# chzchzchz/raftsql

Measured on AMD Instinct MI355X. Metric: quorum decisions/sec (commit+vote) across G groups, higher is better.
Workload: dtype u64

## Files before the change

go/raftq/engine_more.go:

```go
package raftq

import "C"

import "unsafe"

func ABIVersion() int { return int(C.raftq_abi_version()) }

func Quorum(peers uint32) uint32 { return uint32(C.raftq_quorum(C.uint32_t(peers))) }

func (e *Engine) NGroups() uint64 { return uint64(C.raftq_groups(e.h)) }
func (e *Engine) NPeers() uint32  { return uint32(C.raftq_peers(e.h)) }

func (e *Engine) SelfMax() (int, error) {
	var slot C.int32_t
	if err := e.err(C.raftq_self_max(e.h, &slot)); err != nil {
		return -1, err
	}
	return int(slot), nil
}

func (e *Engine) Narrow() (bool, error) {
	var valid C.int32_t
	if err := e.err(C.raftq_narrow(e.h, &valid)); err != nil {
		return false, err
	}
	return valid != 0, nil
}

func (e *Engine) NarrowRebuild() error { return e.err(C.raftq_narrow_rebuild(e.h)) }

func (e *Engine) SetStream(stream unsafe.Pointer) error { return e.err(C.raftq_set_stream(e.h, stream)) }
func (e *Engine) Stream() unsafe.Pointer                { return C.raftq_get_stream(e.h) }

type TermDelta struct{ Group, CurTerm, FirstIdxCurTerm uint64 }

func (e *Engine) ApplyTermDeltas(d []TermDelta) error {
	if len(d) == 0 {
		return nil
	}
	return e.err(C.raftq_apply_term_deltas(e.h, (*C.raftq_term_delta_t)(unsafe.Pointer(&d[0])), C.uint64_t(len(d))))
}

func (e *Engine) CommitAdvance(gated bool, committedOut []uint64) (changed uint64, err error) {
	var p *C.uint64_t
	if committedOut != nil {
		p = (*C.uint64_t)(unsafe.Pointer(&committedOut[0]))
	}
	g := C.int(0)
	if gated {
		g = 1
	}
	var n C.uint64_t
	err = e.err(C.raftq_commit_advance(e.h, g, p, &n))
	return uint64(n), err
}

func (e *Engine) VoteTally(outcomeOut []uint8) (Counts, error) {
	var p *C.uint8_t
	if outcomeOut != nil {
		p = (*C.uint8_t)(unsafe.Pointer(&outcomeOut[0]))
	}
	var c C.raftq_counts_t
	if err := e.err(C.raftq_vote_tally(e.h, p, &c)); err != nil {
		return Counts{}, err
	}
	return Counts{uint64(c.n_changed), uint64(c.n_won), uint64(c.n_lost)}, nil
}

func (e *Engine) ReadVotes(out []uint8) error {
	return e.err(C.raftq_read_votes(e.h, (*C.uint8_t)(unsafe.Pointer(&out[0]))))
}

func (e *Engine) SetTimers(electionTick, heartbeatTick uint32, seed uint64) error {
	return e.err(C.raftq_set_timers(e.h, C.uint32_t(electionTick), C.uint32_t(heartbeatTick), C.uint64_t(seed)))
}

type TickCounts struct{ Hup, Beat uint64 }

func (e *Engine) Tick(wantCounts bool) (TickCounts, error) {
	var c C.raftq_tick_counts_t
	if !wantCounts {
		return TickCounts{}, e.err(C.raftq_tick(e.h, nil))
	}
	err := e.err(C.raftq_tick(e.h, &c))
	return TickCounts{uint64(c.n_hup), uint64(c.n_beat)}, err
}

func (e *Engine) CollectHups(out []uint64) (uint64, error) {
	var n C.uint64_t
	var p *C.uint64_t
	if len(out) > 0 {
		p = (*C.uint64_t)(unsafe.Pointer(&out[0]))
	}
	rc := C.raftq_collect_hups(e.h, p, C.uint64_t(len(out)), &n)
	return uint64(n), e.err(rc)
}

func (e *Engine) TickCollect(hups, beats []uint64) (nHup, nBeat uint64, err error) {
	var hp, bp *C.uint64_t
	if len(hups) > 0 {
		hp = (*C.uint64_t)(unsafe.Pointer(&hups[0]))
	}
	if len(beats) > 0 {
		bp = (*C.uint64_t)(unsafe.Pointer(&beats[0]))
	}
	var nh, nb C.uint64_t
	err = e.err(C.raftq_tick_collect(e.h, hp, C.uint64_t(len(hups)), &nh, bp, C.uint64_t(len(beats)), &nb))
	return uint64(nh), uint64(nb), err
}

const TickBeatBitmap = uint(C.RAFTQ_TICK_BEAT_BITMAP)

// ... 218 lines not shown
```

include/raftq.h:

```cpp
#ifndef RAFTQ_H
#define RAFTQ_H

#include <stddef.h>
#include <stdint.h>

#ifdef __cplusplus
extern "C" {
#endif

#define RAFTQ_ABI_VERSION 1
#define RAFTQ_MAX_PEERS 9

#define RAFTQ_OK 0
#define RAFTQ_EINVAL (-1)
#define RAFTQ_ENOMEM (-2)
#define RAFTQ_EHIP (-3)
#define RAFTQ_ESTATE (-4)
#define RAFTQ_ENODEV (-5)

#define RAFTQ_SWEEP_COMMIT 0x01u
#define RAFTQ_SWEEP_GATED 0x02u
#define RAFTQ_SWEEP_VOTES 0x04u
#define RAFTQ_SWEEP_NO_ADOPT 0x08u
#define RAFTQ_SWEEP_LDS 0x10u
// ... 16 lines not shown
  uint64_t match;
  uint32_t peer;
  uint32_t _pad;
} raftq_delta_t;

typedef struct raftq_vote_delta {
  uint64_t group;
  uint32_t peer;
  uint8_t vote;
  uint8_t _pad[3];
} raftq_vote_delta_t;

typedef struct raftq_term_delta {
  uint64_t group;
  uint64_t cur_term;
  uint64_t first_idx_cur_term;
} raftq_term_delta_t;

typedef struct raftq_advance {
  uint64_t group;
  uint64_t old_commit;
  uint64_t new_commit;
} raftq_advance_t;

typedef struct raftq_delta16 {
  uint64_t match;
  uint32_t group;
  uint32_t peer;
} raftq_delta16_t;
typedef struct raftq_advance16 {
  uint64_t new_commit;
  uint32_t group;
  uint32_t advanced_by;
} raftq_advance16_t;

int raftq_abi_version(void);
int raftq_device_count(int* n);
uint32_t raftq_quorum(uint32_t n_peers);

#define RAFTQ_MAX_GROUPS (1ull << 30)
int raftq_create(int device, uint64_t n_groups, uint32_t n_peers, raftq_t** out);
void raftq_destroy(raftq_t* h);
uint64_t raftq_groups(const raftq_t* h);
uint32_t raftq_peers(const raftq_t* h);
const char* raftq_last_error(const raftq_t* h);

int raftq_set_stream(raftq_t* h, void* stream);
void* raftq_get_stream(const raftq_t* h);

int raftq_load_match(raftq_t* h, const uint64_t* match ,
                     const uint64_t* committed );
int raftq_load_terms(raftq_t* h, const uint64_t* cur_term ,
                     const uint64_t* first_idx_cur_term );
int raftq_load_votes(raftq_t* h, const uint8_t* votes );

int raftq_apply_deltas(raftq_t* h, const raftq_delta_t* d, uint64_t n);
int raftq_apply_vote_deltas(raftq_t* h, const raftq_vote_delta_t* d, uint64_t n);
int raftq_apply_term_deltas(raftq_t* h, const raftq_term_delta_t* d, uint64_t n);

typedef struct raftq_voter_delta {
  uint64_t group;
  uint16_t voters;
  uint16_t reset;
  uint32_t _pad;
} raftq_voter_delta_t;
int raftq_load_voters(raftq_t* h, const uint16_t* voters);
int raftq_apply_voter_deltas(raftq_t* h, const raftq_voter_delta_t* d, uint64_t n);
int raftq_read_voters(raftq_t* h, uint16_t* voters_out);

int raftq_step_async(raftq_t* h, unsigned flags);
int raftq_wait(raftq_t* h, raftq_counts_t* counts);

int raftq_commit_advance(raftq_t* h, int gated, uint64_t* committed_out ,
                         uint64_t* n_changed );
int raftq_vote_tally(raftq_t* h, uint8_t* outcome_out ,
                     raftq_counts_t* counts );

int raftq_read_committed(raftq_t* h, uint64_t* committed_out );
int raftq_read_outcome(raftq_t* h, uint8_t* outcome_out );
int raftq_read_match(raftq_t* h, uint64_t* match_out );
int raftq_self_max(raftq_t* h, int32_t* slot_out);
int raftq_narrow(raftq_t* h, int32_t* valid_out);
int raftq_narrow_rebuild(raftq_t* h);
int raftq_read_votes(raftq_t* h, uint8_t* votes_out );
int raftq_collect_changed(raftq_t* h, raftq_advance_t* out, uint64_t cap, uint64_t* n);

#define RAFTQ_ROLE_FOLLOWER 0
#define RAFTQ_ROLE_CANDIDATE 1
#define RAFTQ_ROLE_LEADER 2
#define RAFTQ_ROLE_PRE_CANDIDATE 3
typedef struct raftq_tick_counts {
  uint64_t n_hup;
  uint64_t n_beat;
} raftq_tick_counts_t;
int raftq_set_timers(raftq_t* h, uint32_t election_tick, uint32_t heartbeat_tick, uint64_t seed);
int raftq_load_roles(raftq_t* h, const uint8_t* role , const uint32_t* elapsed );
int raftq_tick_set_voters(raftq_t* h, int on);
int raftq_tick(raftq_t* h, raftq_tick_counts_t* counts);
int raftq_read_tick(raftq_t* h, uint8_t* action , uint32_t* elapsed , uint8_t* role );
int raftq_collect_hups(raftq_t* h, uint64_t* groups, uint64_t cap, uint64_t* n);
int raftq_collect_beats(raftq_t* h, uint64_t* groups, uint64_t cap, uint64_t* n);
int raftq_tick_collect(raftq_t* h, uint64_t* hups, uint64_t hup_cap, uint64_t* n_hup, uint64_t* beats, uint64_t beat_cap,
                       uint64_t* n_beat);

#define RAFTQ_TICK_BEAT_BITMAP 1u
int raftq_tick_collect_lists(raftq_t* h, unsigned flags, uint64_t hup_cap, uint64_t beat_cap, uint64_t* n_hup, uint64_t* n_beat);
int raftq_last_tick_lists(raftq_t* h, const uint32_t** hups, uint64_t* n_hups, const uint32_t** beats, uint64_t* n_beats,
                          const uint64_t** beat_bitmap, uint64_t* bitmap_words);
int raftq_set_check_quorum(raftq_t* h, int on);
int raftq_tick_set_checks(raftq_t* h, uint64_t chk_cap);
int raftq_last_tick_checks(raftq_t* h, const uint32_t** checks, uint64_t* n_listed, uint64_t* n_total);
int raftq_load_activity(raftq_t* h, const uint16_t* active , const uint32_t* lead_elapsed );
int raftq_read_activity(raftq_t* h, uint16_t* active , uint32_t* lead_elapsed );
int raftq_collect_checks(raftq_t* h, uint64_t* groups, uint64_t cap, uint64_t* n);

int raftq_set_pre_vote(raftq_t* h, int on);

int raftq_set_lead_transfer(raftq_t* h, int on);
int raftq_load_transfer(raftq_t* h, const uint8_t* transferee );
int raftq_read_transfer(raftq_t* h, uint8_t* transferee );

#define RAFTQ_READ_SAFE 1
#define RAFTQ_READ_LEASE 2
int raftq_set_read_index(raftq_t* h, int mode);
int raftq_load_reads(raftq_t* h, const uint32_t* seq , const uint32_t* acked );
int raftq_read_reads(raftq_t* h, uint32_t* seq, uint32_t* acked, uint32_t* confirmed );

int raftq_campaign(raftq_t* h, const uint64_t* groups, uint64_t n, uint32_t self_peer);

int raftq_cycle(raftq_t* h, const raftq_delta_t* deltas, uint64_t n_deltas,
                const raftq_vote_delta_t* vote_deltas, uint64_t n_vote_deltas, unsigned flags,
                raftq_advance_t* advances_out, uint64_t cap, uint64_t* n_advanced,
                raftq_counts_t* counts);

int raftq_stage(raftq_t* h, uint64_t n_deltas, uint64_t n_vote_deltas, raftq_delta_t** deltas,
                raftq_vote_delta_t** vote_deltas);
int raftq_last_advances(raftq_t* h, const raftq_advance_t** list, uint64_t* n_listed);

int raftq_cycle_packed(raftq_t* h, const raftq_delta16_t* deltas, uint64_t n_deltas,
                       const raftq_vote_delta_t* vote_deltas, uint64_t n_vote_deltas, unsigned flags,
                       raftq_advance16_t* advances_out, uint64_t cap, uint64_t* n_advanced,
                       raftq_counts_t* counts);
int raftq_stage_packed(raftq_t* h, uint64_t n_deltas, uint64_t n_vote_deltas, raftq_delta16_t** deltas,
                       raftq_vote_delta_t** vote_deltas);
int raftq_last_advances_packed(raftq_t* h, const raftq_advance16_t** list, uint64_t* n_listed);

#define RAFTQ_CYCLE_SEGMENTED 0x200u
int raftq_last_advance_segments(raftq_t* h, const raftq_advance16_t** recs, const uint32_t** counts, uint32_t* n_segments,
                                uint64_t* stride);

typedef struct raftq_set raftq_set_t;
#define RAFTQ_SET_GRID 0
#define RAFTQ_SET_PERSISTENT 1
int raftq_set_create(raftq_t* const* handles, uint32_t n, raftq_set_t** out);
int raftq_set_create_voters(raftq_t* const* handles, uint32_t n, raftq_set_t** out);
void raftq_set_destroy(raftq_set_t* s);
uint32_t raftq_set_size(const raftq_set_t* s);
const char* raftq_set_last_error(const raftq_set_t* s);
void* raftq_set_get_stream(const raftq_set_t* s);
int raftq_set_mode(raftq_set_t* s, int mode, uint32_t persist_workgroups);
int raftq_set_sweep_async(raftq_set_t* s, unsigned flags);
int raftq_set_tick(raftq_set_t* s);
int raftq_set_wait(raftq_set_t* s, raftq_counts_t* per_member, raftq_counts_t* total);
int raftq_set_timer_begin(raftq_set_t* s);
int raftq_set_timer_end(raftq_set_t* s, float* elapsed_ms);
int raftq_sweep_many_async(raftq_t* const* handles, uint32_t n, unsigned flags);
// ... 13 lines not shown
```

raftsql_amd/_lib.py:

```python
from __future__ import annotations

import ctypes as C
import os

_HERE = os.path.dirname(os.path.abspath(__file__))
LIB_PATH = os.environ.get("RAFTQ_LIB") or os.path.join(_HERE, "libraftq.so")

RAFTQ_OK = 0
RAFTQ_EINVAL, RAFTQ_ENOMEM, RAFTQ_EHIP, RAFTQ_ESTATE, RAFTQ_ENODEV = -1, -2, -3, -4, -5

SWEEP_COMMIT = 0x01
SWEEP_GATED = 0x02
SWEEP_VOTES = 0x04
SWEEP_NO_ADOPT = 0x08
SWEEP_LDS = 0x10
SWEEP_CHANGED = 0x20
SWEEP_STREAM = 0x40
SWEEP_CACHED = 0x80
CYCLE_TRUSTED = 0x100
TICK_BEAT_BITMAP = 1
CYCLE_SEGMENTED = 0x200
SET_GRID, SET_PERSISTENT = 0, 1

MAX_PEERS = 9
READ_SAFE, READ_LEASE = 1, 2


class Counts(C.Structure):
    _fields_ = [("n_changed", C.c_uint64), ("n_won", C.c_uint64), ("n_lost", C.c_uint64)]


class TickCounts(C.Structure):
    _fields_ = [("n_hup", C.c_uint64), ("n_beat", C.c_uint64)]


class Delta(C.Structure):
    _fields_ = [("group", C.c_uint64), ("match", C.c_uint64), ("peer", C.c_uint32), ("_pad", C.c_uint32)]


class VoteDelta(C.Structure):
    _fields_ = [("group", C.c_uint64), ("peer", C.c_uint32), ("vote", C.c_uint8), ("_pad", C.c_uint8 * 3)]


class VoterDelta(C.Structure):
    _fields_ = [("group", C.c_uint64), ("voters", C.c_uint16), ("reset", C.c_uint16), ("_pad", C.c_uint32)]


class Advance(C.Structure):
    _fields_ = [("group", C.c_uint64), ("old_commit", C.c_uint64), ("new_commit", C.c_uint64)]


_H = C.c_void_p
_SIGS = [
    ("raftq_abi_version", C.c_int, []),
    ("raftq_device_count", C.c_int, [C.POINTER(C.c_int)]),
    ("raftq_quorum", C.c_uint32, [C.c_uint32]),
    ("raftq_create", C.c_int, [C.c_int, C.c_uint64, C.c_uint32, C.POINTER(_H)]),
    ("raftq_destroy", None, [_H]),
    ("raftq_groups", C.c_uint64, [_H]),
    ("raftq_peers", C.c_uint32, [_H]),
    ("raftq_last_error", C.c_char_p, [_H]),
    ("raftq_set_stream", C.c_int, [_H, C.c_void_p]),
    ("raftq_get_stream", C.c_void_p, [_H]),
    ("raftq_load_match", C.c_int, [_H, C.c_void_p, C.c_void_p]),
    ("raftq_load_terms", C.c_int, [_H, C.c_void_p, C.c_void_p]),
    ("raftq_load_votes", C.c_int, [_H, C.c_void_p]),
    ("raftq_apply_deltas", C.c_int, [_H, C.c_void_p, C.c_uint64]),
    ("raftq_apply_vote_deltas", C.c_int, [_H, C.c_void_p, C.c_uint64]),
    ("raftq_apply_term_deltas", C.c_int, [_H, C.c_void_p, C.c_uint64]),
    ("raftq_load_voters", C.c_int, [_H, C.c_void_p]),
    ("raftq_apply_voter_deltas", C.c_int, [_H, C.c_void_p, C.c_uint64]),
    ("raftq_read_voters", C.c_int, [_H, C.c_void_p]),
    ("raftq_step_async", C.c_int, [_H, C.c_uint]),
    ("raftq_wait", C.c_int, [_H, C.POINTER(Counts)]),
    ("raftq_commit_advance", C.c_int, [_H, C.c_int, C.c_void_p, C.POINTER(C.c_uint64)]),
    ("raftq_vote_tally", C.c_int, [_H, C.c_void_p, C.POINTER(Counts)]),
    ("raftq_read_committed", C.c_int, [_H, C.c_void_p]),
    ("raftq_read_outcome", C.c_int, [_H, C.c_void_p]),
    ("raftq_read_match", C.c_int, [_H, C.c_void_p]),
    ("raftq_self_max", C.c_int, [_H, C.POINTER(C.c_int32)]),
    ("raftq_narrow", C.c_int, [_H, C.POINTER(C.c_int32)]),
    ("raftq_narrow_rebuild", C.c_int, [_H]),
    ("raftq_read_votes", C.c_int, [_H, C.c_void_p]),
    ("raftq_collect_changed", C.c_int, [_H, C.c_void_p, C.c_uint64, C.POINTER(C.c_uint64)]),
    ("raftq_set_timers", C.c_int, [_H, C.c_uint32, C.c_uint32, C.c_uint64]),
    ("raftq_load_roles", C.c_int, [_H, C.c_void_p, C.c_void_p]),
    ("raftq_tick_set_voters", C.c_int, [_H, C.c_int]),
    ("raftq_tick_set_checks", C.c_int, [_H, C.c_uint64]),
    ("raftq_last_tick_checks", C.c_int, [_H, C.POINTER(C.c_void_p), C.POINTER(C.c_uint64), C.POINTER(C.c_uint64)]),
    ("raftq_tick", C.c_int, [_H, C.POINTER(TickCounts)]),
    ("raftq_read_tick", C.c_int, [_H, C.c_void_p, C.c_void_p, C.c_void_p]),
    ("raftq_collect_hups", C.c_int, [_H, C.c_void_p, C.c_uint64, C.POINTER(C.c_uint64)]),
    ("raftq_collect_beats", C.c_int, [_H, C.c_void_p, C.c_uint64, C.POINTER(C.c_uint64)]),
    ("raftq_tick_collect", C.c_int, [_H, C.c_void_p, C.c_uint64, C.POINTER(C.c_uint64), C.c_void_p, C.c_uint64, C.POINTER(C.c_uint64)]),
    ("raftq_tick_collect_lists", C.c_int, [_H, C.c_uint, C.c_uint64, C.c_uint64, C.POINTER(C.c_uint64), C.POINTER(C.c_uint64)]),
    ("raftq_last_tick_lists", C.c_int, [_H, C.POINTER(C.c_void_p), C.POINTER(C.c_uint64), C.POINTER(C.c_void_p), C.POINTER(C.c_uint64),
                                        C.POINTER(C.c_void_p), C.POINTER(C.c_uint64)]),
    ("raftq_set_check_quorum", C.c_int, [_H, C.c_int]),
    ("raftq_set_pre_vote", C.c_int, [_H, C.c_int]),
    ("raftq_set_lead_transfer", C.c_int, [_H, C.c_int]),
    ("raftq_load_transfer", C.c_int, [_H, C.c_void_p]),
    ("raftq_read_transfer", C.c_int, [_H, C.c_void_p]),
    ("raftq_set_read_index", C.c_int, [_H, C.c_int]),
    ("raftq_load_reads", C.c_int, [_H, C.c_void_p, C.c_void_p]),
    ("raftq_read_reads", C.c_int, [_H, C.c_void_p, C.c_void_p, C.c_void_p]),
    ("raftq_load_activity", C.c_int, [_H, C.c_void_p, C.c_void_p]),
    ("raftq_read_activity", C.c_int, [_H, C.c_void_p, C.c_void_p]),
    ("raftq_collect_checks", C.c_int, [_H, C.c_void_p, C.c_uint64, C.POINTER(C.c_uint64)]),
    ("raftq_campaign", C.c_int, [_H, C.c_void_p, C.c_uint64, C.c_uint32]),
    ("raftq_cycle", C.c_int, [_H, C.c_void_p, C.c_uint64, C.c_void_p, C.c_uint64, C.c_uint, C.c_void_p, C.c_uint64,
                              C.POINTER(C.c_uint64), C.POINTER(Counts)]),
    ("raftq_stage", C.c_int, [_H, C.c_uint64, C.c_uint64, C.POINTER(C.c_void_p), C.POINTER(C.c_void_p)]),
    ("raftq_last_advances", C.c_int, [_H, C.POINTER(C.c_void_p), C.POINTER(C.c_uint64)]),
    ("raftq_cycle_packed", C.c_int, [_H, C.c_void_p, C.c_uint64, C.c_void_p, C.c_uint64, C.c_uint, C.c_void_p, C.c_uint64,
                                     C.POINTER(C.c_uint64), C.POINTER(Counts)]),
    ("raftq_stage_packed", C.c_int, [_H, C.c_uint64, C.c_uint64, C.POINTER(C.c_void_p), C.POINTER(C.c_void_p)]),
    ("raftq_last_advances_packed", C.c_int, [_H, C.POINTER(C.c_void_p), C.POINTER(C.c_uint64)]),
    ("raftq_last_advance_segments", C.c_int, [_H, C.POINTER(C.c_void_p), C.POINTER(C.c_void_p), C.POINTER(C.c_uint32), C.POINTER(C.c_uint64)]),
    ("raftq_set_create", C.c_int, [C.POINTER(_H), C.c_uint32, C.POINTER(_H)]),
    ("raftq_set_create_voters", C.c_int, [C.POINTER(_H), C.c_uint32, C.POINTER(_H)]),
    ("raftq_set_destroy", None, [_H]),
    ("raftq_set_size", C.c_uint32, [_H]),
    ("raftq_set_last_error", C.c_char_p, [_H]),
    ("raftq_set_get_stream", C.c_void_p, [_H]),
    ("raftq_set_mode", C.c_int, [_H, C.c_int, C.c_uint32]),
    ("raftq_set_sweep_async", C.c_int, [_H, C.c_uint]),
    ("raftq_set_wait", C.c_int, [_H, C.c_void_p, C.POINTER(Counts)]),
    ("raftq_set_tick", C.c_int, [_H]),
    ("raftq_set_timer_begin", C.c_int, [_H]),
    ("raftq_set_timer_end", C.c_int, [_H, C.POINTER(C.c_float)]),
    ("raftq_sweep_many_async", C.c_int, [C.POINTER(_H), C.c_uint32, C.c_uint]),
    ("raftq_clone_state", C.c_int, [_H, _H]),
    ("raftq_timer_begin", C.c_int, [_H]),
    ("raftq_timer_end", C.c_int, [_H, C.POINTER(C.c_float)]),
    ("raftq_host_alloc", C.c_int, [C.POINTER(C.c_void_p), C.c_uint64]),
    ("raftq_host_free", None, [C.c_void_p]),
]
EXPORTS = [s[0] for s in _SIGS]


class StepCounts(C.Structure):
    _fields_ = [("n_msgs", C.c_uint64), ("n_groups_touched", C.c_uint64)]


_STEP_SIGS = [
    ("raftq_set_self", C.c_int, [_H, C.c_uint32]),
    ("raftq_load_node", C.c_int, [_H, C.c_void_p, C.c_void_p, C.c_void_p, C.c_void_p, C.c_void_p]),
    ("raftq_read_node", C.c_int, [_H, C.c_void_p, C.c_void_p, C.c_void_p, C.c_void_p, C.c_void_p, C.c_void_p]),
    ("raftq_step_batch", C.c_int, [_H, C.c_void_p, C.c_uint64, C.c_void_p, C.POINTER(StepCounts)]),
    ("raftq_apply_log_deltas", C.c_int, [_H, C.c_void_p, C.c_uint64, C.c_void_p]),
    ("raftq_apply_log_deltas_nowait", C.c_int, [_H, C.c_void_p, C.c_uint64]),
    ("raftq_step_submit", C.c_int, [_H, C.c_void_p, C.c_uint64]),
    ("raftq_step_collect", C.c_int, [_H, C.c_void_p, C.POINTER(StepCounts)]),
    ("raftq_step_stage", C.c_int, [_H, C.c_uint64, C.POINTER(C.c_void_p)]),
    ("raftq_step_stage_packed", C.c_int, [_H, C.c_uint64, C.POINTER(C.c_void_p)]),
    ("raftq_step_submit_packed", C.c_int, [_H, C.c_void_p, C.c_uint64]),
    ("raftq_step_results", C.c_int, [_H, C.POINTER(C.c_void_p), C.POINTER(C.c_uint64)]),
    ("raftq_step_set_compact", C.c_int, [_H, C.c_int]),
    ("raftq_step_set_msg_flags", C.c_int, [_H, C.c_int]),
    ("raftq_step_set_voters", C.c_int, [_H, C.c_int]),
    ("raftq_step_set_props", C.c_int, [_H, C.c_int]),
    ("raftq_step_results_c", C.c_int, [_H, C.POINTER(C.c_void_p), C.POINTER(C.c_uint64)]),
    ("raftq_step_results_s", C.c_int, [_H, C.POINTER(C.c_void_p), C.POINTER(C.c_uint64)]),
]
STEP_EXPORTS = [s[0] for s in _STEP_SIGS]
# ... 86 lines not shown
```

raftsql_amd/csrc/raftq_capi.hip:

```cpp
#include "raftq.h"

#include <hip/hip_runtime.h>

#include <algorithm>
#include <atomic>
#include <mutex>
#include <chrono>
#include <cstdlib>
#include <cstdio>
#include <cstring>
#include <new>
#include <string>
#include <type_traits>
#include <unordered_set>
#include <vector>

#include "raftq_internal.hpp"

#ifndef RAFTQ_GPL
#define RAFTQ_GPL 4
#endif
#ifndef RAFTQ_AUTO_STREAM_BYTES
#define RAFTQ_AUTO_STREAM_BYTES (128ull << 20)
#endif
// ... 56 lines not shown
    case 6: return f(Const<6>{});
    case 7: return f(Const<7>{});
    case 8: return f(Const<8>{});
    case 9: return f(Const<9>{});
    default: return hipErrorInvalidValue;
  }
}

template <class F>
hipError_t with_flag_form(unsigned flags, F f) {
  const bool commit = flags & (RAFTQ_SWEEP_COMMIT | RAFTQ_SWEEP_GATED);
  const bool gated = flags & RAFTQ_SWEEP_GATED;
  const bool votes = flags & RAFTQ_SWEEP_VOTES;
  if (commit && gated) return votes ? f(FlagForm<true, true, true>{}) : f(FlagForm<true, true, false>{});
  if (commit) return votes ? f(FlagForm<true, false, true>{}) : f(FlagForm<true, false, false>{});
  return f(FlagForm<false, false, true>{});
}

template <class F>
hipError_t with_policy(int nt, F f) {
  if (nt == 3) return f(Const<kLdNT | kStNT>{});
  if (nt == 1) return f(Const<kLdNT>{});
  return f(Const<0>{});
}

constexpr int set_gpl(int n_peers) { return n_peers <= 5 ? 8 : 2; }

template <int N, class Form, int POLICY>
hipError_t launch_reg(const SweepLaunch& L, hipStream_t s) {
  constexpr bool COMMIT = Form::commit, GATED = Form::gated, VOTES = Form::votes;
  const unsigned tiles = (unsigned)(L.gpad / kTile);
  if (L.tab == nullptr) {
    hipLaunchKernelGGL((sweep_kernel<N, kGPL, COMMIT, GATED, VOTES, POLICY, true>), dim3(tiles), dim3(kBlock), 0, s, *L.one);
  } else if (L.persist_wgs == 0) {
    constexpr int G = set_gpl(N);
    hipLaunchKernelGGL((sweep_set_kernel<N, G, COMMIT, GATED, VOTES, POLICY, true>),
                       dim3((unsigned)(L.gpad / ((uint64_t)kBlock * G)), L.members), dim3(kBlock), 0, s, L.tab, L.want_bits);
  } else {
    const uint32_t total = tiles * L.members;
    hipLaunchKernelGGL((sweep_persist_kernel<N, kGPL, COMMIT, GATED, VOTES, POLICY, true>),
                       dim3(std::min<uint32_t>(L.persist_wgs, total)), dim3(kBlock), 0, s, L.tab, tiles, total, L.want_bits);
  }
  return hipGetLastError();
}

template <int N, class Form>
hipError_t launch_lds(const SweepArgs& a, uint64_t gpad, hipStream_t s) {
  if constexpr (Form::commit) {
    constexpr uint64_t tile = (uint64_t)kBlock * kLdsGPL;
    constexpr int rows = N + 1 + (Form::gated ? 1 : 0);
    constexpr size_t lds = (size_t)kWaves * (kLdsGPL / 2) * rows * 1024;
    const dim3 grid((unsigned)(gpad / tile));
    hipLaunchKernelGGL((sweep_lds_kernel<N, kLdsGPL, Form::gated, Form::votes, true>), grid, dim3(kBlock), lds, s, a);
    return hipGetLastError();
  } else {
    return hipErrorInvalidValue;
  }
}

hipError_t launch_sweep(uint32_t N, const SweepLaunch& L, unsigned flags, int nt, hipStream_t s) {
  const bool lds = (flags & RAFTQ_SWEEP_LDS) && (flags & (RAFTQ_SWEEP_COMMIT | RAFTQ_SWEEP_GATED));
  if (lds && L.tab) return hipErrorInvalidValue;
  return with_peers(N, [&](auto n) {
    return with_flag_form(flags, [&](auto form) {
      if (lds) return launch_lds<decltype(n)::value, decltype(form)>(*L.one, L.gpad, s);
      return with_policy(nt, [&](auto pol) { return launch_reg<decltype(n)::value, decltype(form), decltype(pol)::value>(L, s); });
    });
  });
}

hipError_t launch_segments(uint32_t N, const SweepArgs& a, uint32_t n_tiles, bool gated, int nt, Advance16* list, unsigned int* counts_host,
                           unsigned int* counts_dev, hipStream_t s) {
  const dim3 grid(n_tiles), block(kBlock);
  return with_peers(N, [&](auto n) {
    return with_policy(nt, [&](auto pol) {
      constexpr int NP = decltype(n)::value, POLICY = decltype(pol)::value;
      if (gated) hipLaunchKernelGGL((sweep_segments_kernel<NP, kGPL, true, POLICY>), grid, block, 0, s, a, list, counts_host, counts_dev);
      else hipLaunchKernelGGL((sweep_segments_kernel<NP, kGPL, false, POLICY>), grid, block, 0, s, a, list, counts_host, counts_dev);
      return hipGetLastError();
    });
  });
}

constexpr int voters_gpl(int n_peers) { return n_peers <= 6 ? 4 : 2; }

hipError_t launch_voters(uint32_t N, const VoterSweepArgs& a, uint64_t gpad, unsigned flags, int nt, hipStream_t s) {
  return with_peers(N, [&](auto n) {
    return with_flag_form(flags, [&](auto form) {
      return with_policy(nt, [&](auto pol) {
        using Form = decltype(form);
        constexpr int NP = decltype(n)::value, G = voters_gpl(NP);
        const dim3 grid((unsigned)(gpad / ((uint64_t)kBlock * G))), block(kBlock);
        hipLaunchKernelGGL((sweep_voters_kernel<NP, G, Form::commit, Form::gated, Form::votes, decltype(pol)::value>), grid, block, 0, s, a);
        return hipGetLastError();
      });
    });
  });
}

struct VoterSetLaunch {
  const VoterSweepArgs* tab;
  uint32_t members, want_bits;
  uint64_t gpad;
};

hipError_t launch_set_voters(uint32_t N, const VoterSetLaunch& L, unsigned flags, int nt, hipStream_t s) {
  return with_peers(N, [&](auto n) {
    return with_flag_form(flags, [&](auto form) {
      return with_policy(nt, [&](auto pol) {
        using Form = decltype(form);
        constexpr int NP = decltype(n)::value, G = voters_gpl(NP);
        const dim3 grid((unsigned)(L.gpad / ((uint64_t)kBlock * G)), L.members), block(kBlock);
        hipLaunchKernelGGL((sweep_set_voters_kernel<NP, G, Form::commit, Form::gated, Form::votes, decltype(pol)::value>), grid, block, 0, s,
                           L.tab, L.want_bits);
        return hipGetLastError();
      });
    });
  });
}

}
static inline void dense_changed(raftq_t* h) { h->node_mirror_fresh = false; }

int raftq_detail::ensure_staging(raftq_t* h, size_t bytes) {
  HIPCHK(h, h->stage.grow(bytes, std::max({bytes, h->stage.cap * 2, (size_t)1 << 20}), &h->stream));
  return RAFTQ_OK;
}

int raftq_detail::ensure_ingest(raftq_t* h, size_t bytes) {
  HIPCHK(h, h->ingest.grow(bytes, std::max({bytes, h->ingest.cap * 2, (size_t)1 << 20}), &h->stream, h->bar));
  return RAFTQ_OK;
}

namespace {
int ensure_adv(raftq_t* h, uint64_t entries) {
  const uint64_t have = h->adv.cap / sizeof(Advance);
  const uint64_t want = std::min<uint64_t>(std::max<uint64_t>({entries, have * 2, 4096}), h->gpad);
  HIPCHK(h, h->adv.grow(entries * sizeof(Advance), want * sizeof(Advance), &h->stream));
  return RAFTQ_OK;
}

}
int raftq_detail::self_max_check(raftq_t* h) {
  if (int rc = use_device(h)) return rc;
  if (h->step_collected != h->step_submitted) {
    HIPCHK(h, hipMemsetAsync(h->self_max, 0, sizeof(uint32_t), h->stream));
    return RAFTQ_OK;
  }
  HIPCHK(h, hipMemsetD32Async((hipDeviceptr_t)h->self_max, (int)(kSelfMaxValid | h->self_peer), 1, h->stream));
  const uint64_t blocks = std::min<uint64_t>((h->G + kBlock - 1) / kBlock, 4096);
  hipLaunchKernelGGL(self_max_check_kernel, dim3((unsigned)std::max<uint64_t>(blocks, 1)), dim3(kBlock), 0, h->stream,
                     (const uint64_t*)h->match, h->ld, h->G, h->N, h->self_peer, h->self_max);
  HIPCHK(h, hipGetLastError());
  return RAFTQ_OK;
}
int raftq_detail::narrow_build(raftq_t* h) {
  if (int rc = use_device(h)) return rc;
  if (h->narrow_off) return RAFTQ_OK;
  if (h->step_collected != h->step_submitted) {
    HIPCHK(h, hipMemsetAsync(h->narrow_word(), 0, sizeof(uint32_t), h->stream));
    return RAFTQ_OK;
  }
  if (!h->anchor) {
    const hipError_t e = raftq_buf::alloc_group({{(void**)&h->anchor, h->ld * sizeof(uint64_t)},
                                                 {(void**)&h->moff, (size_t)h->N * h->ld * sizeof(uint32_t)}},
                                                h->stream);
    if (e != hipSuccess) {
      (void)hipGetLastError();
      return RAFTQ_OK;
    }
    if (h->in_set) h->in_set->tab_stale = true;
  }
  HIPCHK(h, hipMemsetD32Async((hipDeviceptr_t)h->narrow_word(), (int)kNarrowValid, 1, h->stream));
  const uint64_t blocks = std::min<uint64_t>((h->G + kBlock - 1) / kBlock, 4096);
  hipLaunchKernelGGL(narrow_build_kernel, dim3((unsigned)std::max<uint64_t>(blocks, 1)), dim3(kBlock), 0, h->stream,
                     (const uint64_t*)h->match, h->ld, h->G, h->N, h->anchor, h->moff, h->narrow_word());
  HIPCHK(h, hipGetLastError());
  return RAFTQ_OK;
}
int raftq_detail::use_device(raftq_t* h) {
  if (!h) return fail(nullptr, RAFTQ_EINVAL, "null handle");
  HIPCHK(h, hipSetDevice(h->device));
  return RAFTQ_OK;
}
int raftq_detail::use_device_idle(raftq_t* h, const char* who) {
  if (int rc = use_device(h)) return rc;
  if (h->step_collected != h->step_submitted)
    return fail(h, RAFTQ_ESTATE, std::string(who) + ": Step batches are in flight; collect them first");
  return RAFTQ_OK;
}
using raftq_detail::ensure_staging;
using raftq_detail::ensure_ingest;
using raftq_detail::use_device;
using raftq_detail::use_device_idle;
using raftq_detail::ensure_tick_state;

template <typename W>
static void pack_votes(const uint8_t* votes, uint64_t G, uint32_t N, W* out) {
  for (uint64_t g = 0; g < G; ++g) out[g] = 0;
  for (uint32_t p = 0; p < N; ++p) {
    const uint8_t* row = votes + (size_t)p * G;
    for (uint64_t g = 0; g < G; ++g) {
      const uint8_t v = row[g];
      out[g] = (W)(out[g] | (W)((v == 1 ? 1u : v == 2 ? 2u : 0u) << (2 * p)));
    }
  }
}
template <typename W>
static void unpack_votes(const W* in, uint64_t G, uint32_t N, uint8_t* votes) {
  for (uint32_t p = 0; p < N; ++p) {
    uint8_t* row = votes + (size_t)p * G;
    for (uint64_t g = 0; g < G; ++g) {
      const uint32_t f = ((uint32_t)in[g] >> (2 * p)) & 3u;
      row[g] = f == 3u ? 0 : (uint8_t)f;
    }
  }
}

extern "C" {

int raftq_abi_version(void) { return RAFTQ_ABI_VERSION; }

uint32_t raftq_quorum(uint32_t n_peers) { return n_peers / 2 + 1; }

int raftq_device_count(int* n) {
  if (!n) return fail(nullptr, RAFTQ_EINVAL, "raftq_device_count: null out");
  int c = 0;
  hipError_t e = hipGetDeviceCount(&c);
  if (e != hipSuccess) {
    *n = 0;
    return fail(nullptr, RAFTQ_ENODEV, std::string("hipGetDeviceCount: ") + hipGetErrorString(e));
  }
  *n = c;
  return RAFTQ_OK;
}

const char* raftq_last_error(const raftq_t* h) { return h ? h->err.c_str() : g_err.c_str(); }

uint64_t raftq_groups(const raftq_t* h) { return h ? h->G : 0; }
uint32_t raftq_peers(const raftq_t* h) { return h ? h->N : 0; }

int raftq_create(int device, uint64_t n_groups, uint32_t n_peers, raftq_t** out) {
  if (!out) return fail(nullptr, RAFTQ_EINVAL, "raftq_create: null out");
  *out = nullptr;
  if (n_groups == 0 || n_groups > RAFTQ_MAX_GROUPS)
    return fail(nullptr, RAFTQ_EINVAL, "raftq_create: n_groups out of range (1 .. RAFTQ_MAX_GROUPS = 2^30 per handle)");
  if (n_peers < 1 || n_peers > RAFTQ_MAX_PEERS) return fail(nullptr, RAFTQ_EINVAL, "raftq_create: n_peers must be 1..9");
  int ndev = 0;
  if (hipGetDeviceCount(&ndev) != hipSuccess || ndev <= 0)
    return fail(nullptr, RAFTQ_ENODEV, "raftq_create: no HIP device (this library has no CPU path)");
  if (device < 0 || device >= ndev) return fail(nullptr, RAFTQ_ENODEV, "raftq_create: device index out of range");
  raftq_t* h = new (std::nothrow) raftq();
  if (!h) return fail(nullptr, RAFTQ_ENOMEM, "raftq_create: host allocation failed");
  h->device = device;
  h->G = n_groups;
  h->N = n_peers;
  h->last_gpl = kGPL;
  h->gpad = (n_groups + kTileMax - 1) / kTileMax * kTileMax;
  h->ld = h->gpad + kRowStagger;
  const uint64_t ld = h->ld;
  h->max_partials = h->gpad / (kBlock * 2) * kWaves;
  int rc = RAFTQ_OK;
  do {
    if ((rc = use_device(h))) break;
    hipError_t e = hipStreamCreateWithFlags(&h->stream, hipStreamNonBlocking);
    if (e != hipSuccess) { rc = fail(h, RAFTQ_EHIP, std::string("hipStreamCreate: ") + hipGetErrorString(e)); break; }
    h->own_stream = true;
    {
      int large_bar = 0;
      (void)hipDeviceGetAttribute(&large_bar, hipDeviceAttributeIsLargeBar, device);
      const char* st = std::getenv("RAFTQ_STAGE");
      h->bar.staging = large_bar == 1 && !(st && std::strcmp(st, "host") == 0);
    }
    e = raftq_buf::alloc_group({{(void**)&h->match, (size_t)n_peers * ld * 8},
                                {(void**)&h->committed[0], ld * 8},
                                {(void**)&h->committed[1], ld * 8},
                                {(void**)&h->first_idx, ld * 8},
                                {(void**)&h->votes, (size_t)vote_word_bytes((int)n_peers) * ld},
                                {(void**)&h->outcome, ld / 4 + 64},
                                {(void**)&h->changed_bits, h->gpad / 8},
                                {(void**)&h->partials, h->max_partials * sizeof(uint4)},
                                {(void**)&h->offsets, (h->max_partials + 1) * 8},
                                {(void**)&h->self_max, 64}},
                               h->stream);
    if (e != hipSuccess) {
      rc = fail(h, e == hipErrorOutOfMemory ? RAFTQ_ENOMEM : RAFTQ_EHIP, std::string("device arrays: ") + hipGetErrorString(e));
      break;
    }
    {
      const char* nr = std::getenv("RAFTQ_NARROW");
      h->narrow_off = nr && std::strcmp(nr, "0") == 0;
    }
    e = hipMemsetD32Async((hipDeviceptr_t)h->self_max, (int)(kSelfMaxValid | 0u), 1, h->stream);
    if (e != hipSuccess) { rc = fail(h, RAFTQ_EHIP, std::string("hipMemsetD32Async: ") + hipGetErrorString(e)); break; }
    e = raftq_buf::alloc_group({{(void**)&h->h_partials, h->max_partials * sizeof(uint4), raftq_buf::Kind::pinned},
                                {(void**)&h->h_total, 64, raftq_buf::Kind::mapped_coherent, (void**)&h->d_total}},
                               h->stream);
    if (e != hipSuccess) { rc = fail(h, RAFTQ_ENOMEM, std::string("page-locked memory: ") + hipGetErrorString(e)); break; }
    e = hipEventCreate(&h->ev0);
    if (e == hipSuccess) e = hipEventCreate(&h->ev1);
    if (e != hipSuccess) { rc = fail(h, RAFTQ_EHIP, std::string("hipEventCreate: ") + hipGetErrorString(e)); break; }
    e = hipStreamSynchronize(h->stream);
    if (e != hipSuccess) { rc = fail(h, RAFTQ_EHIP, std::string("hipStreamSynchronize: ") + hipGetErrorString(e)); break; }
  } while (0);
  if (rc != RAFTQ_OK) {
    std::string keep = h->err;
    raftq_destroy(h);
    g_err = keep;
    return rc;
  }
  *out = h;
  return RAFTQ_OK;
}

void raftq_destroy(raftq_t* h) {
  if (!h) return;
  if (h->in_set) {
    raftq_set_t* s = h->in_set;
    s->broken = true;
    s->members.erase(std::remove(s->members.begin(), s->members.end(), h), s->members.end());
    (void)hipSetDevice(h->device);
    (void)hipStreamSynchronize(s->stream);
    h->stream = nullptr;
    h->own_stream = false;
  }
  if (h->prof_n && std::getenv("RAFTQ_PROFILE"))
    std::fprintf(stderr,
                 "[raftq] cycle phases, avg us over %llu calls: stage/validate %.1f | enqueue scatter %.1f | enqueue sweep "
                 "%.1f | enqueue collect %.1f | sync %.1f | copy-out %.1f | turns that ended in the blocking wait instead of the "
                 "polled flag: %llu\n",
                 (unsigned long long)h->prof_n, h->prof[0] / h->prof_n, h->prof[1] / h->prof_n, h->prof[2] / h->prof_n,
                 h->prof[3] / h->prof_n, h->prof[4] / h->prof_n, h->prof[5] / h->prof_n, (unsigned long long)h->flag_fallbacks);
  (void)hipSetDevice(h->device);
  if (h->stream) (void)hipStreamSynchronize(h->stream);
  if (h->many_aux) (void)hipStreamSynchronize(h->many_aux);
  raftq_detail::free_node_state(h);
  raftq_detail::free_wire_state(h);
  raftq_buf::free_device(h->match, h->committed[0], h->committed[1], h->first_idx, h->votes, h->voters, h->outcome, h->changed_bits,
                         h->partials, h->offsets, h->self_max, h->anchor, h->moff, h->claim, h->delta_bad, h->role, h->elapsed, h->action, h->hup_bits,
                         h->beat_bits, h->tick_partials, h->tick_offsets2, h->tick_offsets3, h->cq, h->chk_bits, h->reads);
  raftq_buf::free_host(h->h_partials, h->h_total);
  if (h->ev0) (void)hipEventDestroy(h->ev0);
  if (h->ev1) (void)hipEventDestroy(h->ev1);
  if (h->many_aux) {
    (void)hipEventDestroy(h->many_fork);
    (void)hipEventDestroy(h->many_join);
  }
  const hipStream_t streams[4] = {h->many_aux, h->step_s_in, h->step_s_out, h->own_stream ? h->stream : nullptr};
  delete h;
  for (hipStream_t st : streams)
    if (st) (void)hipStreamDestroy(st);
}

int raftq_set_stream(raftq_t* h, void* stream) {
  if (int rc = use_device_idle(h, "raftq_set_stream")) return rc;
  if (h->in_set) return fail(h, RAFTQ_ESTATE, "raftq_set_stream: the handle is a member of a sweep set, which owns its stream");
  HIPCHK(h, hipStreamSynchronize(h->stream));
  if (h->own_stream) HIPCHK(h, hipStreamDestroy(h->stream));
  h->stream = (hipStream_t)stream;
  h->own_stream = false;
  return RAFTQ_OK;
}

void* raftq_get_stream(const raftq_t* h) { return h ? (void*)h->stream : nullptr; }

int raftq_load_match(raftq_t* h, const uint64_t* match, const uint64_t* committed) {
  if (int rc = use_device_idle(h, "raftq_load_match")) return rc;
  if (!match && !committed) return fail(h, RAFTQ_EINVAL, "raftq_load_match: nothing to load");
  if (match) {
    for (uint32_t p = 0; p < h->N; ++p)
      HIPCHK(h, hipMemcpyAsync(h->match + (size_t)p * h->ld, match + (size_t)p * h->G, h->G * 8, hipMemcpyHostToDevice, h->stream));
    if (int rc = raftq_detail::self_max_check(h)) return rc;
    if (int rc = raftq_detail::narrow_build(h)) return rc;
  }
  dense_changed(h);
  if (committed)
    HIPCHK(h, hipMemcpyAsync(h->committed[h->cur], committed, h->G * 8, hipMemcpyHostToDevice, h->stream));
  HIPCHK(h, hipStreamSynchronize(h->stream));
  return RAFTQ_OK;
}

int raftq_load_terms(raftq_t* h, const uint64_t* cur_term, const uint64_t* first_idx_cur_term) {
  if (int rc = use_device_idle(h, "raftq_load_terms")) return rc;
  if (!cur_term || !first_idx_cur_term) return fail(h, RAFTQ_EINVAL, "raftq_load_terms: null argument");
  std::vector<uint64_t> f;
  try {
    f.assign(first_idx_cur_term, first_idx_cur_term + h->G);
  } catch (...) {
    return fail(h, RAFTQ_ENOMEM, "raftq_load_terms: host allocation failed");
  }
  for (uint64_t g = 0; g < h->G; ++g)
    if (cur_term[g] == 0) f[g] = 0;
  HIPCHK(h, hipMemcpyAsync(h->first_idx, f.data(), h->G * 8, hipMemcpyHostToDevice, h->stream));
  dense_changed(h);
  HIPCHK(h, hipStreamSynchronize(h->stream));
  h->have_terms = true;
  return RAFTQ_OK;
}

int raftq_load_votes(raftq_t* h, const uint8_t* votes) {
  if (int rc = use_device_idle(h, "raftq_load_votes")) return rc;
  if (!votes) return fail(h, RAFTQ_EINVAL, "raftq_load_votes: null argument");
  const size_t wb = (size_t)vote_word_bytes((int)h->N);
  std::vector<uint8_t> packed;
  try {
    packed.resize(h->G * wb);
  } catch (...) {
    return fail(h, RAFTQ_ENOMEM, "raftq_load_votes: host allocation failed");
  }
  if (wb == 2) pack_votes(votes, h->G, h->N, reinterpret_cast<uint16_t*>(packed.data()));
  else pack_votes(votes, h->G, h->N, reinterpret_cast<uint32_t*>(packed.data()));
  HIPCHK(h, hipMemcpyAsync(h->votes, packed.data(), packed.size(), hipMemcpyHostToDevice, h->stream));
  HIPCHK(h, hipStreamSynchronize(h->stream));
  return RAFTQ_OK;
}

static int ensure_delta_dev(raftq_t* h, size_t bytes) {
  if (!h->delta_bad) HIPCHK(h, raftq_buf::alloc_zeroed((void**)&h->delta_bad, 64, h->stream));
  HIPCHK(h, h->delta_dev.grow(bytes, std::max(bytes * 2, (size_t)1 << 20), &h->stream));
  return RAFTQ_OK;
}

static int check_deltas(raftq_t* h, bool trusted = false) {
  int rc = RAFTQ_OK;
  const char* what = trusted ? "; that record was dropped, every other record of the turn was applied (RAFTQ_CYCLE_TRUSTED)"
                             : "; nothing applied";
  if (h->delta_check[0] && h->h_total[1] == h->delta_check[0])
    rc = fail(h, RAFTQ_EINVAL, std::string("a match delta is out of range (group >= G or peer >= N)") + what);
  if (h->delta_check[1] && h->h_total[2] == h->delta_check[1])
    rc = fail(h, RAFTQ_EINVAL, std::string("a vote delta is invalid (group/peer out of range or vote not 1/2)") + what);
  h->delta_check[0] = h->delta_check[1] = 0;
  return rc;
}

}

template <typename Rec, typename AbiRec>
static int enqueue_ingest(raftq_t* h, const AbiRec* d, uint64_t n, const raftq_vote_delta_t* vd, uint64_t nv, size_t off_votes,
                          bool trusted = false) {
  static_assert(sizeof(Rec) == sizeof(AbiRec), "ABI struct mismatch");
  static_assert(sizeof(VoteDeltaRec) == sizeof(raftq_vote_delta_t), "ABI struct mismatch");
  if (nv > 0xfffffffeull) return fail(h, RAFTQ_EINVAL, "vote delta batch too large");
  auto inside = [&](const void* q) {
    return (const uint8_t*)q >= (const uint8_t*)h->ingest.h && (const uint8_t*)q < (const uint8_t*)h->ingest.h + h->ingest.cap;
  };
  if (n) {
    AbiRec* dst = (AbiRec*)h->ingest.h;
    if ((const void*)d != (const void*)dst) {
      if (inside(d)) return fail(h, RAFTQ_EINVAL, "match deltas staged with other counts / another record layout than this call's");
      std::memcpy(dst, d, (size_t)n * sizeof(AbiRec));
    }
  }
  if (nv) {
    raftq_vote_delta_t* dst = (raftq_vote_delta_t*)((uint8_t*)h->ingest.h + off_votes);
    if ((const void*)vd != (const void*)dst) {
      if (inside(vd)) return fail(h, RAFTQ_EINVAL, "vote deltas staged with other counts / another record layout than this call's");
      std::memcpy(dst, vd, (size_t)nv * sizeof(raftq_vote_delta_t));
    }
    if (!h->claim) {
      HIPCHK(h, raftq_buf::alloc_filled((void**)&h->claim, (size_t)h->N * h->ld * sizeof(uint32_t), 0xff, h->stream));
    }
  }
  h->ingest.publish();
  if (int rc = ensure_delta_dev(h, h->ingest.cap)) return rc;
  const unsigned long long em = n ? ++h->delta_epoch : kNoEpoch, ev = nv ? ++h->delta_epoch : kNoEpoch;
  h->delta_check[0] = n ? em : 0;
  h->delta_check[1] = nv ? ev : 0;
  Rec* dev_m = (Rec*)h->delta_dev.d;
  VoteDeltaRec* dev_v = (VoteDeltaRec*)((uint8_t*)h->delta_dev.d + off_votes);
  const unsigned long long* bad = h->delta_bad;
  const dim3 gm((unsigned)((n + kBlock - 1) / kBlock)), gv((unsigned)((nv + kBlock - 1) / kBlock));
  if (n) dense_changed(h);
  if (n && trusted)
    hipLaunchKernelGGL((deltas_in_apply_kernel<Rec>), gm, dim3(kBlock), 0, h->stream, (const Rec*)h->ingest.d, n, h->match, h->ld,
                       h->G, h->N, h->delta_bad, h->d_total + 1, em, h->self_max, h->narrow_mirror());
  else if (n)
    hipLaunchKernelGGL((deltas_in_kernel<Rec>), gm, dim3(kBlock), 0, h->stream, (const Rec*)h->ingest.d, dev_m, n, h->G, h->N,
                       h->delta_bad, h->d_total + 1, em);
  if (nv)
    hipLaunchKernelGGL(vote_deltas_in_kernel, gv, dim3(kBlock), 0, h->stream,
                       (const VoteDeltaRec*)((uint8_t*)h->ingest.d + off_votes), dev_v, nv, h->G, h->N, h->delta_bad + 1,
                       h->d_total + 2, ev);
  if (n && !trusted)
    hipLaunchKernelGGL((apply_deltas_kernel<Rec>), gm, dim3(kBlock), 0, h->stream, h->match, h->ld, (const Rec*)dev_m, n, bad, em,
                       ev, h->self_max, h->narrow_mirror());
  if (nv) {
    const unsigned long long em_gate = trusted ? kNoEpoch : em;
    hipLaunchKernelGGL(vote_claim_kernel, gv, dim3(kBlock), 0, h->stream, h->claim, h->ld, (const VoteDeltaRec*)dev_v, nv, bad,
                       em_gate, ev, h->G, h->N, trusted ? 1 : 0);
    hipLaunchKernelGGL(vote_apply_kernel, gv, dim3(kBlock), 0, h->stream, h->votes, h->N > 8 ? 1 : 0, h->claim, h->ld,
                       (const VoteDeltaRec*)dev_v, nv, bad, em_gate, ev, h->G, h->N, trusted ? 1 : 0);
  }
  HIPCHK(h, hipGetLastError());
  return RAFTQ_OK;
}

extern "C" {

int raftq_apply_deltas(raftq_t* h, const raftq_delta_t* d, uint64_t n) {
  if (int rc = use_device_idle(h, "raftq_apply_deltas")) return rc;
  if (n == 0) return RAFTQ_OK;
  if (!d) return fail(h, RAFTQ_EINVAL, "raftq_apply_deltas: null argument");
  if (int rc = ensure_ingest(h, (size_t)n * sizeof(raftq_delta_t))) return rc;
  if (int rc = enqueue_ingest<DeltaRec>(h, d, n, nullptr, 0, 0)) return rc;
  HIPCHK(h, hipStreamSynchronize(h->stream));
  return check_deltas(h);
}

int raftq_apply_term_deltas(raftq_t* h, const raftq_term_delta_t* d, uint64_t n) {
  static_assert(sizeof(TermDeltaRec) == sizeof(raftq_term_delta_t), "ABI struct mismatch");
  if (int rc = use_device_idle(h, "raftq_apply_term_deltas")) return rc;
  if (n == 0) return RAFTQ_OK;
  if (!d) return fail(h, RAFTQ_EINVAL, "raftq_apply_term_deltas: null argument");
  for (uint64_t i = 0; i < n; ++i)
    if (d[i].group >= h->G) return fail(h, RAFTQ_EINVAL, "a term delta is out of range; nothing applied");
  if (int rc = ensure_staging(h, (size_t)n * sizeof(raftq_term_delta_t))) return rc;
  raftq_term_delta_t* dst = (raftq_term_delta_t*)h->stage.h;
  uint64_t m = 0;
  {
    std::unordered_set<uint64_t> seen;
    seen.reserve((size_t)n * 2);
    std::vector<uint64_t> keep;
    keep.reserve(n);
    for (uint64_t i = n; i-- > 0;)
      if (seen.insert(d[i].group).second) keep.push_back(i);
    for (auto it = keep.rbegin(); it != keep.rend(); ++it) dst[m++] = d[*it];
  }
  const dim3 grid((unsigned)((m + kBlock - 1) / kBlock));
  dense_changed(h);
  hipLaunchKernelGGL(apply_term_deltas_kernel, grid, dim3(kBlock), 0, h->stream, h->first_idx,
                     (const TermDeltaRec*)h->stage.d, m);
  HIPCHK(h, hipGetLastError());
  HIPCHK(h, hipStreamSynchronize(h->stream));
  h->have_terms = true;
  return RAFTQ_OK;
}

int raftq_apply_vote_deltas(raftq_t* h, const raftq_vote_delta_t* d, uint64_t n) {
  if (int rc = use_device_idle(h, "raftq_apply_vote_deltas")) return rc;
  if (n == 0) return RAFTQ_OK;
  if (!d) return fail(h, RAFTQ_EINVAL, "raftq_apply_vote_deltas: null argument");
  if (int rc = ensure_ingest(h, (size_t)n * sizeof(raftq_vote_delta_t))) return rc;
  if (int rc = enqueue_ingest<DeltaRec>(h, (const raftq_delta_t*)nullptr, 0, d, n, 0)) return rc;
  HIPCHK(h, hipStreamSynchronize(h->stream));
  return check_deltas(h);
}

}

static int ensure_voters(raftq_t* h) {
  if (h->voters) return RAFTQ_OK;
  HIPCHK(h, raftq_buf::alloc_zeroed((void**)&h->voters, h->ld * sizeof(uint16_t), h->stream));
  if (h->in_set) h->in_set->tab_stale = true;
  return RAFTQ_OK;
}
static int drop_voters(raftq_t* h) {
  if (!h->voters) return RAFTQ_OK;
  HIPCHK(h, hipStreamSynchronize(h->stream));
  raftq_buf::free_device(h->voters);
  if (h->in_set) h->in_set->tab_stale = true;
  return RAFTQ_OK;
}
static int voters_not_in_set(raftq_t* h, const char* who) {
  if (!h->in_set || h->in_set->allow_voters) return RAFTQ_OK;
  return fail(h, RAFTQ_ESTATE, std::string(who) + ": the handle is a member of a sweep set, whose dispatches count every slot "
                                                  "(voter masks on set members are out of scope)");
}
int raftq_detail::refuse_voters(raftq_t* h, const char* who, bool step_family, bool tick_rounds, bool bcast) {
// ... 48 lines not shown
  if (n == 0) return RAFTQ_OK;
  if (!d) return fail(h, RAFTQ_EINVAL, "raftq_apply_voter_deltas: null argument");
  const uint32_t beyond = 0xffffu & ~((1u << h->N) - 1u);
  for (uint64_t i = 0; i < n; ++i)
    if (d[i].group >= h->G || ((d[i].voters | d[i].reset) & beyond))
      return fail(h, RAFTQ_EINVAL, "a voter delta is out of range (group >= G or a bit >= N); nothing applied");
  if (int rc = ensure_staging(h, (size_t)n * sizeof(raftq_voter_delta_t))) return rc;
  raftq_voter_delta_t* dst = (raftq_voter_delta_t*)h->stage.h;
  uint64_t m = 0;
  try {
    std::unordered_set<uint64_t> seen;
    seen.reserve((size_t)n * 2);
    std::vector<uint64_t> keep;
    keep.reserve(n);
    for (uint64_t i = n; i-- > 0;)
      if (seen.insert(d[i].group).second) keep.push_back(i);
    for (auto it = keep.rbegin(); it != keep.rend(); ++it) dst[m++] = d[*it];
  } catch (...) {
    return fail(h, RAFTQ_ENOMEM, "raftq_apply_voter_deltas: host allocation failed");
  }
  if (!h->voters) {
    if (int rc = ensure_voters(h)) return rc;
    hipLaunchKernelGGL(fill_voters_kernel, dim3((unsigned)((h->G + kBlock - 1) / kBlock)), dim3(kBlock), 0, h->stream, h->voters, h->G,
                       (uint16_t)((1u << h->N) - 1u));
    HIPCHK(h, hipGetLastError());
  }
  dense_changed(h);
  hipLaunchKernelGGL(apply_voter_deltas_kernel, dim3((unsigned)((m + kBlock - 1) / kBlock)), dim3(kBlock), 0, h->stream, h->voters, h->match,
                     h->ld, h->votes, h->N > 8 ? 1 : 0, h->N, (const VoterDeltaRec*)h->stage.d, m, h->self_max, h->narrow_word());
  HIPCHK(h, hipGetLastError());
  HIPCHK(h, hipStreamSynchronize(h->stream));
  return RAFTQ_OK;
}

static int sweep_check(raftq_t* h, unsigned flags, const char* who) {
  const unsigned known = RAFTQ_SWEEP_COMMIT | RAFTQ_SWEEP_GATED | RAFTQ_SWEEP_VOTES | RAFTQ_SWEEP_NO_ADOPT |
                         RAFTQ_SWEEP_LDS | RAFTQ_SWEEP_CHANGED | RAFTQ_SWEEP_STREAM | RAFTQ_SWEEP_CACHED;
  const std::string w(who);
  if (flags & ~known) return fail(h, RAFTQ_EINVAL, w + ": unknown flag");
  const bool commit = flags & (RAFTQ_SWEEP_COMMIT | RAFTQ_SWEEP_GATED);
  const bool votes = flags & RAFTQ_SWEEP_VOTES;
  if (!commit && !votes) return fail(h, RAFTQ_EINVAL, w + ": nothing to sweep");
  if ((flags & RAFTQ_SWEEP_GATED) && !h->have_terms)
    return fail(h, RAFTQ_ESTATE, w + ": gated sweep before raftq_load_terms");
  if ((flags & RAFTQ_SWEEP_STREAM) && (flags & RAFTQ_SWEEP_CACHED))
    return fail(h, RAFTQ_EINVAL, w + ": RAFTQ_SWEEP_STREAM and RAFTQ_SWEEP_CACHED are exclusive");
  if ((flags & RAFTQ_SWEEP_CHANGED) && !commit)
    return fail(h, RAFTQ_EINVAL, w + ": RAFTQ_SWEEP_CHANGED needs a commit sweep");
  if ((flags & RAFTQ_SWEEP_LDS) && h->voters)
    return fail(h, RAFTQ_EINVAL, w + ": RAFTQ_SWEEP_LDS has no form for a handle with voter masks loaded (the A/B variant counts every slot)");
  return RAFTQ_OK;
}

static SweepArgs sweep_args(const raftq_t* h, int cur, bool want_bits) {
  SweepArgs a;
  a.match = h->match;
  a.committed = h->committed[cur];
  a.committed_out = h->committed[cur ^ 1];
  a.first_idx = h->first_idx;
  a.votes = h->votes;
  a.outcome = h->outcome;
  a.changed_bits = want_bits ? h->changed_bits : nullptr;
  a.partials = h->partials;
  a.ld = h->ld;
  a.self_max = h->self_max;
  a.narrow = h->anchor ? h->narrow_word() : nullptr;
  a.anchor = h->anchor;
  a.moff = h->moff;
  return a;
}

static uint64_t sweep_footprint(const raftq_t* h) { return h->ld * (8ull * h->N + 24 + vote_word_bytes((int)h->N) + 1 + (h->voters ? 2 : 0)); }

static int sweep_policy(unsigned flags, uint64_t footprint) {
  const bool stream = (flags & RAFTQ_SWEEP_STREAM) ? true
                      : (flags & RAFTQ_SWEEP_CACHED) ? false
                                                     : footprint >= RAFTQ_AUTO_STREAM_BYTES;
  return !stream ? 0 : footprint >= RAFTQ_AUTO_STREAM_BYTES ? 3 : 1;
}

static void sweep_done(raftq_t* h, unsigned flags, int gpl) {
  const bool commit = flags & (RAFTQ_SWEEP_COMMIT | RAFTQ_SWEEP_GATED);
  h->n_partials = h->gpad / ((uint64_t)kBlock * gpl) * kWaves;
  h->last_flags = flags;
  h->last_gpl = gpl;
  if (commit) {
    h->last_old = h->committed[h->cur];
    h->last_new = h->committed[h->cur ^ 1];
    if (!(flags & RAFTQ_SWEEP_NO_ADOPT)) {
      h->cur ^= 1;
      dense_changed(h);
    }
  }
}

static int sweep_on(raftq_t* h, unsigned flags, hipStream_t s, const char* who) {
  if (int rc = use_device_idle(h, who)) return rc;
  if (int rc = sweep_check(h, flags, who)) return rc;
  const bool commit = flags & (RAFTQ_SWEEP_COMMIT | RAFTQ_SWEEP_GATED);
  const SweepArgs a = sweep_args(h, h->cur, flags & RAFTQ_SWEEP_CHANGED);
  if (h->voters) {
    VoterSweepArgs va;
    va.s = a;
    va.voters = h->voters;
    HIPCHK(h, launch_voters(h->N, va, h->gpad, flags, sweep_policy(flags, sweep_footprint(h)), s));
    sweep_done(h, flags, voters_gpl((int)h->N));
    return RAFTQ_OK;
  }
  const bool lds = (flags & RAFTQ_SWEEP_LDS) && commit;
  SweepLaunch L;
  L.one = &a;
  L.gpad = h->gpad;
  HIPCHK(h, launch_sweep(h->N, L, flags, sweep_policy(flags, sweep_footprint(h)), s));
  sweep_done(h, flags, lds ? kLdsGPL : kGPL);
  return RAFTQ_OK;
}

int raftq_step_async(raftq_t* h, unsigned flags) {
  if (!h) return fail(nullptr, RAFTQ_EINVAL, "null handle");
  return sweep_on(h, flags, h->stream, "raftq_step_async");
}


int raftq_sweep_many_async(raftq_t* const* handles, uint32_t n, unsigned flags) {
  if (!handles && n) return fail(nullptr, RAFTQ_EINVAL, "raftq_sweep_many_async: null handle array");
  bool alternate = n >= 2;
  for (uint32_t i = 0; alternate && i < n; ++i) {
    if (!handles[i] || handles[i]->stream != handles[0]->stream || handles[i]->device != handles[0]->device) alternate = false;
    for (uint32_t j = 0; alternate && j < i; ++j)
      if (handles[j] == handles[i]) alternate = false;
  }
  if (!alternate) {
    for (uint32_t i = 0; i < n; ++i)
      if (int rc = raftq_step_async(handles[i], flags)) return rc;
    return RAFTQ_OK;
  }
  raftq_t* h0 = handles[0];
  if (int rc = use_device(h0)) return rc;
  if (!h0->many_aux) {
    HIPCHK(h0, hipStreamCreateWithFlags(&h0->many_aux, hipStreamNonBlocking));
    HIPCHK(h0, hipEventCreateWithFlags(&h0->many_fork, hipEventDisableTiming));
    HIPCHK(h0, hipEventCreateWithFlags(&h0->many_join, hipEventDisableTiming));
  }
  HIPCHK(h0, hipEventRecord(h0->many_fork, h0->stream));
  HIPCHK(h0, hipStreamWaitEvent(h0->many_aux, h0->many_fork, 0));
  int rc = RAFTQ_OK;
  for (uint32_t i = 0; i < n && rc == RAFTQ_OK; ++i)
    rc = sweep_on(handles[i], flags, (i & 1) ? h0->many_aux : h0->stream, "raftq_sweep_many_async");
  HIPCHK(h0, hipEventRecord(h0->many_join, h0->many_aux));
  HIPCHK(h0, hipStreamWaitEvent(h0->stream, h0->many_join, 0));
  return rc;
}

int raftq_wait(raftq_t* h, raftq_counts_t* counts) {
  if (int rc = use_device_idle(h, "raftq_wait")) return rc;
  if (counts) {
    if (h->n_partials == 0) return fail(h, RAFTQ_ESTATE, "raftq_wait: no sweep to report on");
    HIPCHK(h, hipMemcpyAsync(h->h_partials, h->partials, h->n_partials * sizeof(uint4), hipMemcpyDeviceToHost, h->stream));
  }
  HIPCHK(h, hipStreamSynchronize(h->stream));
  if (counts) {
    uint64_t c = 0, w = 0, l = 0;
    for (uint64_t i = 0; i < h->n_partials; ++i) {
      c += h->h_partials[i].x;
      w += h->h_partials[i].y;
      l += h->h_partials[i].z;
    }
    const bool commit = h->last_flags & (RAFTQ_SWEEP_COMMIT | RAFTQ_SWEEP_GATED);
    const bool votes = h->last_flags & RAFTQ_SWEEP_VOTES;
    counts->n_changed = commit ? c : 0;
    counts->n_won = votes ? w : 0;
    counts->n_lost = votes ? l : 0;
  }
  return RAFTQ_OK;
}

int raftq_read_committed(raftq_t* h, uint64_t* out) {
  if (int rc = use_device_idle(h, "raftq_read_committed")) return rc;
  if (!out) return fail(h, RAFTQ_EINVAL, "raftq_read_committed: null argument");
  const uint64_t* src = (h->last_flags & RAFTQ_SWEEP_NO_ADOPT) && h->last_new ? h->last_new : h->committed[h->cur];
  HIPCHK(h, hipMemcpyAsync(out, src, h->G * 8, hipMemcpyDeviceToHost, h->stream));
  HIPCHK(h, hipStreamSynchronize(h->stream));
  return RAFTQ_OK;
}

int raftq_read_outcome(raftq_t* h, uint8_t* out) {
  if (int rc = use_device_idle(h, "raftq_read_outcome")) return rc;
  if (!out) return fail(h, RAFTQ_EINVAL, "raftq_read_outcome: null argument");
  std::vector<uint8_t> packed;
  try {
    packed.resize((h->G + 3) / 4);
  } catch (...) {
    return fail(h, RAFTQ_ENOMEM, "raftq_read_outcome: host allocation failed");
  }
  HIPCHK(h, hipMemcpyAsync(packed.data(), h->outcome, packed.size(), hipMemcpyDeviceToHost, h->stream));
  HIPCHK(h, hipStreamSynchronize(h->stream));
  for (uint64_t g = 0; g < h->G; ++g) out[g] = (uint8_t)((packed[g >> 2] >> (2 * (g & 3))) & 3u);
  return RAFTQ_OK;
}

int raftq_self_max(raftq_t* h, int32_t* slot) {
  if (int rc = use_device_idle(h, "raftq_self_max")) return rc;
  if (!slot) return fail(h, RAFTQ_EINVAL, "raftq_self_max: null argument");
  uint32_t w = 0;
  HIPCHK(h, hipMemcpyAsync(&w, h->self_max, sizeof w, hipMemcpyDeviceToHost, h->stream));
  HIPCHK(h, hipStreamSynchronize(h->stream));
  *slot = (w & kSelfMaxValid) ? (int32_t)(w & 0xffu) : -1;
  return RAFTQ_OK;
}

int raftq_narrow(raftq_t* h, int32_t* valid) {
  if (int rc = use_device_idle(h, "raftq_narrow")) return rc;
  if (!valid) return fail(h, RAFTQ_EINVAL, "raftq_narrow: null argument");
  uint32_t w = 0;
  HIPCHK(h, hipMemcpyAsync(&w, h->narrow_word(), sizeof w, hipMemcpyDeviceToHost, h->stream));
  HIPCHK(h, hipStreamSynchronize(h->stream));
  *valid = w == kNarrowValid ? 1 : 0;
  return RAFTQ_OK;
}

int raftq_narrow_rebuild(raftq_t* h) {
  if (int rc = use_device_idle(h, "raftq_narrow_rebuild")) return rc;
  if (int rc = raftq_detail::narrow_build(h)) return rc;
  HIPCHK(h, hipStreamSynchronize(h->stream));
  return RAFTQ_OK;
}

int raftq_read_match(raftq_t* h, uint64_t* out) {
  if (int rc = use_device_idle(h, "raftq_read_match")) return rc;
  if (!out) return fail(h, RAFTQ_EINVAL, "raftq_read_match: null argument");
  for (uint32_t p = 0; p < h->N; ++p)
    HIPCHK(h, hipMemcpyAsync(out + (size_t)p * h->G, h->match + (size_t)p * h->ld, h->G * 8, hipMemcpyDeviceToHost, h->stream));
  HIPCHK(h, hipStreamSynchronize(h->stream));
  return RAFTQ_OK;
}

int raftq_read_votes(raftq_t* h, uint8_t* out) {
  if (int rc = use_device_idle(h, "raftq_read_votes")) return rc;
  if (!out) return fail(h, RAFTQ_EINVAL, "raftq_read_votes: null argument");
  const size_t wb = (size_t)vote_word_bytes((int)h->N);
  std::vector<uint8_t> packed;
  try {
    packed.resize(h->G * wb);
  } catch (...) {
    return fail(h, RAFTQ_ENOMEM, "raftq_read_votes: host allocation failed");
  }
  HIPCHK(h, hipMemcpyAsync(packed.data(), h->votes, packed.size(), hipMemcpyDeviceToHost, h->stream));
  HIPCHK(h, hipStreamSynchronize(h->stream));
  if (wb == 2) unpack_votes(reinterpret_cast<const uint16_t*>(packed.data()), h->G, h->N, out);
  else unpack_votes(reinterpret_cast<const uint32_t*>(packed.data()), h->G, h->N, out);
  return RAFTQ_OK;
}

int raftq_commit_advance(raftq_t* h, int gated, uint64_t* committed_out, uint64_t* n_changed) {
  if (int rc = raftq_step_async(h, gated ? (RAFTQ_SWEEP_COMMIT | RAFTQ_SWEEP_GATED) : RAFTQ_SWEEP_COMMIT)) return rc;
  raftq_counts_t c;
  if (int rc = raftq_wait(h, &c)) return rc;
  if (n_changed) *n_changed = c.n_changed;
  if (committed_out) return raftq_read_committed(h, committed_out);
  return RAFTQ_OK;
}

int raftq_vote_tally(raftq_t* h, uint8_t* outcome_out, raftq_counts_t* counts) {
  if (int rc = raftq_step_async(h, RAFTQ_SWEEP_VOTES)) return rc;
  raftq_counts_t c;
  if (int rc = raftq_wait(h, &c)) return rc;
  if (counts) *counts = c;
  if (outcome_out) return raftq_read_outcome(h, outcome_out);
  return RAFTQ_OK;
}

}

int raftq_detail::ensure_tick_state(raftq_t* h) {
  if (h->role) return RAFTQ_OK;
  HIPCHK(h, raftq_buf::alloc_group({{(void**)&h->role, h->ld},
                                    {(void**)&h->elapsed, h->ld * 4},
                                    {(void**)&h->action, h->ld},
                                    {(void**)&h->hup_bits, h->gpad / 8},
                                    {(void**)&h->beat_bits, h->gpad / 8},
                                    {(void**)&h->tick_partials, h->gpad / 256 * sizeof(uint4)}},
                                   h->stream));
  return RAFTQ_OK;
}

int raftq_detail::refuse_check_quorum(raftq_t* h, const char* who, bool fused) {
  if (!h->cq || (fused && h->tick_chk_cap != 0)) return RAFTQ_OK;
  return fail(h, RAFTQ_ESTATE, std::string(who) + ": raftq_set_check_quorum is on (check quorum): this call's beat lists and device-built rounds do not "
                                                  "know a beat suppressed by a failing check -- use raftq_tick with raftq_collect_hups / _beats / _checks");
}
int raftq_detail::refuse_pre_vote(raftq_t* h, const char* who, bool fused) {
  if (!h->pre_vote || (fused && h->tick_chk_cap != 0)) return RAFTQ_OK;
  return fail(h, RAFTQ_ESTATE, std::string(who) + ": raftq_set_pre_vote is on (pre vote): this call's device-built round makes a MsgHup a becomeCandidate and "
                                                  "sends MsgVote -- step the MsgHup (RAFTQ_OUT_PRE_CAMPAIGN) and send MsgPreVote");
}
int raftq_detail::refuse_lead_transfer(raftq_t* h, const char* who) {
  if (!h->lead_transfer) return RAFTQ_OK;
  return fail(h, RAFTQ_ESTATE, std::string(who) + ": raftq_set_lead_transfer is on (lead transfer): a leader drops its own proposals while a transfer is "
                                                  "pending, and this call's kernels do not read the word that says so");
}
// ... 613 lines not shown

int raftq_collect_beats(raftq_t* h, uint64_t* groups, uint64_t cap, uint64_t* n) {
  return collect_tick_list(h, "raftq_collect_beats", 1, groups, cap, n);
}

int raftq_collect_checks(raftq_t* h, uint64_t* groups, uint64_t cap, uint64_t* n) {
  if (h && !h->cq) {
    if (int rc = use_device_idle(h, "raftq_collect_checks")) return rc;
    if (!n) return fail(h, RAFTQ_EINVAL, "raftq_collect_checks: null count");
    if (cap && !groups) return fail(h, RAFTQ_EINVAL, "raftq_collect_checks: null out with cap > 0");
    *n = 0;
    return RAFTQ_OK;
  }
  return collect_tick_list(h, "raftq_collect_checks", 2, groups, cap, n);
}

int raftq_campaign(raftq_t* h, const uint64_t* groups, uint64_t n, uint32_t self_peer) {
  if (int rc = use_device_idle(h, "raftq_campaign")) return rc;
  if (n == 0) return RAFTQ_OK;
  if (!groups) return fail(h, RAFTQ_EINVAL, "raftq_campaign: null argument");
  if (self_peer >= h->N) return fail(h, RAFTQ_EINVAL, "raftq_campaign: self_peer out of range");
  uint64_t bad = 0;
  for (uint64_t i = 0; i < n; ++i) bad |= (uint64_t)(groups[i] >= h->G);
  if (bad) return fail(h, RAFTQ_EINVAL, "raftq_campaign: a group is out of range; nothing applied");
  if (int rc = ensure_tick_state(h)) return rc;
  if (int rc = ensure_staging(h, (size_t)n * 8)) return rc;
  std::memcpy(h->stage.h, groups, n * 8);
  hipLaunchKernelGGL(campaign_kernel, dim3((unsigned)((n + kBlock - 1) / kBlock)), dim3(kBlock), 0, h->stream,
                     h->role, h->elapsed, h->votes, h->N, self_peer, (const uint64_t*)h->stage.d, n);
  dense_changed(h);
  HIPCHK(h, hipGetLastError());
  HIPCHK(h, hipStreamSynchronize(h->stream));
  return RAFTQ_OK;
}

}


template <typename Adv>
static int enqueue_collect(raftq_t* h, uint64_t take_cap, bool want_flag) {
  static_assert(sizeof(Advance) == sizeof(raftq_advance_t) && sizeof(Advance16) == sizeof(raftq_advance16_t), "ABI struct mismatch");
  const int gpl = h->last_gpl;
  const dim3 grid((unsigned)(h->gpad / ((uint64_t)kBlock * gpl)));
  Adv* out = (Adv*)h->adv.d;
  const uint64_t* wave_offsets = nullptr;
  if (h->n_partials > (1u << 14)) {
    hipLaunchKernelGGL(scan_partials_kernel, dim3(1), dim3(1024), 0, h->stream, h->partials, h->n_partials, h->offsets,
                       h->d_total, 0);
    wave_offsets = h->offsets;
  }
  switch (gpl) {
    case 2:
      hipLaunchKernelGGL((compact_changed_kernel<2, Adv>), grid, dim3(kBlock), 0, h->stream, h->changed_bits, h->partials,
                         h->last_old, h->last_new, out, take_cap, h->d_total, wave_offsets);
      break;
    case 8:
      hipLaunchKernelGGL((compact_changed_kernel<8, Adv>), grid, dim3(kBlock), 0, h->stream, h->changed_bits, h->partials,
                         h->last_old, h->last_new, out, take_cap, h->d_total, wave_offsets);
      break;
    default:
      static_assert((kGPL == 4 || kGPL == 8) && kLdsGPL == 4, "compaction instantiations cover GPL 2, 4, 8");
      hipLaunchKernelGGL((compact_changed_kernel<4, Adv>), grid, dim3(kBlock), 0, h->stream, h->changed_bits, h->partials,
                         h->last_old, h->last_new, out, take_cap, h->d_total, wave_offsets);
  }
  HIPCHK(h, hipGetLastError());
  h->compact_epoch_armed = 0;
  if (want_flag) {
    const uint64_t epoch = ++h->compact_epoch;
    hipLaunchKernelGGL(raise_flag_kernel, dim3(1), dim3(64), 0, h->stream, h->d_total + 3, epoch);
    HIPCHK(h, hipGetLastError());
    h->compact_epoch_armed = epoch;
  }
  return RAFTQ_OK;
}

constexpr uint64_t kSegmentsMaxGroups = 1ull << 22;
static bool segments_ok(const raftq_t* h, unsigned flags) {
  if (const char* e = std::getenv("RAFTQ_CYCLE_SEGMENTS"))
    if (e[0] == '0') return false;
  const unsigned allowed = RAFTQ_SWEEP_COMMIT | RAFTQ_SWEEP_GATED | RAFTQ_SWEEP_CHANGED | RAFTQ_SWEEP_NO_ADOPT | RAFTQ_SWEEP_STREAM | RAFTQ_SWEEP_CACHED;
  if (h->voters) return false;
  return (flags & (RAFTQ_SWEEP_COMMIT | RAFTQ_SWEEP_GATED)) && !(flags & ~allowed) && h->gpad <= kSegmentsMaxGroups;
}
static int enqueue_sweep_segments(raftq_t* h, unsigned flags) {
  const uint32_t n_tiles = (uint32_t)(h->gpad / kTile);
  if (int rc = ensure_adv(h, (h->gpad * sizeof(Advance16) + sizeof(Advance) - 1) / sizeof(Advance))) return rc;
  HIPCHK(h, h->seg_h.grow((size_t)n_tiles * 4, (size_t)n_tiles * 4, &h->stream));
  HIPCHK(h, h->seg_d.grow((size_t)n_tiles * 4, (size_t)n_tiles * 4, &h->stream));
  const SweepArgs a = sweep_args(h, h->cur, true);
  uint64_t epoch = ++h->compact_epoch;
  if ((uint32_t)epoch == 0) epoch = ++h->compact_epoch;
  HIPCHK(h, launch_segments(h->N, a, n_tiles, (flags & RAFTQ_SWEEP_GATED) != 0, sweep_policy(flags, sweep_footprint(h)), (Advance16*)h->adv.d, h->seg_h.d,
                            h->seg_d.d, h->stream));
  sweep_done(h, flags, kGPL);
  hipLaunchKernelGGL(raise_flag_segments_kernel, dim3(1), dim3(kBlock), 0, h->stream, h->d_total + 3, (uint32_t)epoch, h->seg_d.d, n_tiles);
  HIPCHK(h, hipGetLastError());
  h->compact_epoch_armed = (uint64_t)(uint32_t)epoch << 32;
  h->flag_mask = 0xffffffff00000000ull;
  h->seg_tiles = n_tiles;
  h->seg_stride = kTile;
  return RAFTQ_OK;
}

extern "C" {

int raftq_collect_changed(raftq_t* h, raftq_advance_t* out, uint64_t cap, uint64_t* n) {
  if (int rc = use_device_idle(h, "raftq_collect_changed")) return rc;
  if (!n) return fail(h, RAFTQ_EINVAL, "raftq_collect_changed: null count");
  if (!(h->last_flags & RAFTQ_SWEEP_CHANGED) || !h->last_old)
    return fail(h, RAFTQ_ESTATE, "raftq_collect_changed: last sweep did not set RAFTQ_SWEEP_CHANGED");
  if (cap && !out) return fail(h, RAFTQ_EINVAL, "raftq_collect_changed: null out with cap > 0");
  const uint64_t take_cap = std::min<uint64_t>(cap, h->G);
  if (take_cap)
    if (int rc = ensure_adv(h, take_cap)) return rc;
  if (int rc = enqueue_collect<Advance>(h, take_cap, false)) return rc;
  HIPCHK(h, hipStreamSynchronize(h->stream));
  const uint64_t total = *h->h_total;
  *n = total;
  const uint64_t take = std::min(total, take_cap);
  h->adv_listed = take;
  h->adv_packed = false;
  h->adv_segmented = false;
  if (take) std::memcpy(out, h->adv.h, take * sizeof(Advance));
  return RAFTQ_OK;
}

static size_t vote_stage_offset(uint64_t n_deltas) {
  return ((size_t)n_deltas * sizeof(raftq_delta_t) + 255) / 256 * 256;
}

int raftq_stage(raftq_t* h, uint64_t n_deltas, uint64_t n_vote_deltas, raftq_delta_t** deltas,
                raftq_vote_delta_t** vote_deltas) {
  if (int rc = use_device_idle(h, "raftq_stage")) return rc;
  const size_t off_votes = vote_stage_offset(n_deltas);
  if (int rc = ensure_ingest(h, off_votes + (size_t)n_vote_deltas * sizeof(raftq_vote_delta_t) + 256)) return rc;
  if (deltas) *deltas = (raftq_delta_t*)h->ingest.h;
  if (vote_deltas) *vote_deltas = (raftq_vote_delta_t*)((uint8_t*)h->ingest.h + off_votes);
  return RAFTQ_OK;
}

int raftq_last_advances(raftq_t* h, const raftq_advance_t** list, uint64_t* n_listed) {
  if (!h) return fail(nullptr, RAFTQ_EINVAL, "null handle");
  if (!list || !n_listed) return fail(h, RAFTQ_EINVAL, "raftq_last_advances: null argument");
  if (h->adv_listed && h->adv_packed)
    return fail(h, RAFTQ_ESTATE, "raftq_last_advances: the last list was produced in the packed layout");
  *list = (const raftq_advance_t*)h->adv.h;
  *n_listed = h->adv_listed;
  return RAFTQ_OK;
}

}

static hipError_t wait_turn(raftq_t* h, uint64_t flag_epoch, int kind) {
  constexpr uint32_t kMisses = 8, kRetry = 1024;
  const bool try_flag = flag_epoch && (h->flag_misses[kind] < kMisses || (++h->flag_rested[kind] % kRetry) == 0);
  if (try_flag) {
    volatile uint64_t* flag = h->h_total + 3;
    const auto t0 = std::chrono::steady_clock::now();
    for (int i = 0;; ++i) {
      if ((*flag & h->flag_mask) == flag_epoch) {
        std::atomic_thread_fence(std::memory_order_acquire);
        h->flag_misses[kind] = 0;
        if (hipPeekAtLastError() == hipSuccess) return hipSuccess;
        (void)hipGetLastError();
        return hipStreamSynchronize(h->stream);
      }
      if ((i & 255) == 255 && std::chrono::steady_clock::now() - t0 > std::chrono::microseconds(2000)) break;
    }
    ++h->flag_misses[kind];
  }
  if (flag_epoch) ++h->flag_fallbacks;
  return hipStreamSynchronize(h->stream);
}

hipError_t raftq_detail::wait_call(raftq_t* h) {
  hipError_t e;
  if (!h->d_total) {
    e = hipStreamSynchronize(h->stream);
  } else {
    const uint64_t epoch = ++h->compact_epoch;
    h->flag_mask = ~0ull;
    hipLaunchKernelGGL(raise_flag_kernel, dim3(1), dim3(64), 0, h->stream, h->d_total + 3, epoch);
    e = hipGetLastError() != hipSuccess ? hipStreamSynchronize(h->stream) : wait_turn(h, epoch, 1);
  }
  if (e == hipSuccess && h->wal_pending && !h->wal_pending_done) h->wal_pending_waited = true;
  return e;
}

template <typename Rec, typename Adv, typename AbiRec, typename AbiAdv>
static int cycle_impl(raftq_t* h, const char* who, const AbiRec* deltas, uint64_t n_deltas, const raftq_vote_delta_t* vote_deltas,
                      uint64_t n_vote_deltas, unsigned flags, AbiAdv* advances_out, uint64_t cap, uint64_t* n_advanced,
                      raftq_counts_t* counts) {
  if (int rc = use_device_idle(h, who)) return rc;
  if ((n_deltas && !deltas) || (n_vote_deltas && !vote_deltas))
    return fail(h, RAFTQ_EINVAL, std::string(who) + ": null array with non-zero length");
  const bool want_segments = (flags & RAFTQ_CYCLE_SEGMENTED) != 0;
  flags &= ~RAFTQ_CYCLE_SEGMENTED;
  if (int rc = sweep_check(h, flags & ~RAFTQ_CYCLE_TRUSTED, who)) return rc;
  const bool commit = flags & (RAFTQ_SWEEP_COMMIT | RAFTQ_SWEEP_GATED);
  const bool want_list = commit && (advances_out || n_advanced || cap);
  if (want_list) flags |= RAFTQ_SWEEP_CHANGED;
  const size_t off_votes = ((size_t)n_deltas * sizeof(AbiRec) + 255) / 256 * 256;
  {
    const size_t need = off_votes + (size_t)n_vote_deltas * sizeof(raftq_vote_delta_t) + 256;
    auto staged = [&](const void* q) {
      return q && h->ingest.h && (const uint8_t*)q >= (const uint8_t*)h->ingest.h &&
             (const uint8_t*)q < (const uint8_t*)h->ingest.h + h->ingest.cap;
    };
    if (need > h->ingest.cap && (staged(deltas) || staged(vote_deltas)))
      return fail(h, RAFTQ_EINVAL, std::string(who) + ": the staged arrays were sized for fewer records than this call names");
    if (int rc = ensure_ingest(h, need)) return rc;
  }
  const uint64_t take_cap = want_list ? std::min<uint64_t>(cap, h->G) : 0;
  if (take_cap)
    if (int rc = ensure_adv(h, take_cap)) return rc;
  using clk = std::chrono::steady_clock;
  auto us = [](clk::time_point a, clk::time_point b) { return std::chrono::duration<double, std::micro>(b - a).count(); };
  const auto t0 = clk::now();
  const bool trusted = flags & RAFTQ_CYCLE_TRUSTED;
  flags &= ~RAFTQ_CYCLE_TRUSTED;
  if (n_deltas || n_vote_deltas)
    if (int rc = enqueue_ingest<Rec>(h, deltas, n_deltas, vote_deltas, n_vote_deltas, off_votes, trusted)) return rc;
  const auto t1 = clk::now();
  const int cur_before = h->cur;
  const bool flag_wake = want_list && !counts;
  const bool segmented = want_segments && flag_wake && !advances_out && sizeof(Adv) == sizeof(Advance16) && segments_ok(h, flags);
  h->flag_mask = ~0ull;
  h->adv_segmented = false;
  if (segmented) {
    if (int rc = enqueue_sweep_segments(h, flags | RAFTQ_SWEEP_CHANGED)) return rc;
  } else if (int rc = raftq_step_async(h, flags)) {
    return rc;
  }
  const auto t2 = clk::now();
  if (want_list && !segmented)
    if (int rc = enqueue_collect<Adv>(h, take_cap, flag_wake)) return rc;
  if (counts)
    HIPCHK(h, hipMemcpyAsync(h->h_partials, h->partials, h->n_partials * sizeof(uint4), hipMemcpyDeviceToHost,
                             h->stream));
  const auto t3 = clk::now();
  HIPCHK(h, wait_turn(h, flag_wake ? h->compact_epoch_armed : 0));
  if (flag_wake && h->compact_epoch_armed) {
    static const bool check = [] { const char* e = std::getenv("RAFTQ_CYCLE_CHECK"); return e && e[0] == '1'; }();
    if (check) {
      auto digest = [&]() {
        const volatile uint64_t* w = (const volatile uint64_t*)h->adv.h;
        if (segmented) {
          uint64_t d = (h->h_total[3] & 0xffffffffull) * 0x9E3779B97F4A7C15ull;
          for (uint32_t t = 0; t < h->seg_tiles; ++t) {
            const uint32_t c = ((const volatile uint32_t*)h->seg_h.h)[t];
            d = (d ^ c) * 0xBF58476D1CE4E5B9ull;
            for (uint64_t i = 0; i < (uint64_t)c * 2; ++i) d = (d ^ w[(uint64_t)t * h->seg_stride * 2 + i]) * 0xBF58476D1CE4E5B9ull;
          }
          return d;
        }
        const uint64_t total = *h->h_total;
        const uint64_t words = std::min(total, take_cap) * (sizeof(Adv) / 8);
        uint64_t d = total * 0x9E3779B97F4A7C15ull;
        for (uint64_t i = 0; i < words; ++i) d = (d ^ w[i]) * 0xBF58476D1CE4E5B9ull;
        return d;
      };
      const uint64_t at_flag = digest();
      HIPCHK(h, hipStreamSynchronize(h->stream));
      if (digest() != at_flag)
        return fail(h, RAFTQ_EHIP, std::string(who) + ": the completion flag arrived before the advance list it announces "
                                                      "(RAFTQ_CYCLE_CHECK)");
    }
  }
  const auto t4 = clk::now();
  h->prof[1] += us(t0, t1);
  h->prof[2] += us(t1, t2);
  h->prof[3] += us(t2, t3);
  h->prof[4] += us(t3, t4);
  h->prof_n++;
  const int verdict = check_deltas(h, trusted);
  if (verdict != RAFTQ_OK && !trusted) {
    h->cur = cur_before;
    dense_changed(h);
    if (n_advanced) *n_advanced = 0;
    if (counts) *counts = raftq_counts_t{0, 0, 0};
    h->adv_listed = 0;
    return verdict;
  }
  if (counts) {
    uint64_t c = 0, w = 0, l = 0;
    for (uint64_t i = 0; i < h->n_partials; ++i) {
      c += h->h_partials[i].x;
      w += h->h_partials[i].y;
      l += h->h_partials[i].z;
    }
    counts->n_changed = commit ? c : 0;
    counts->n_won = (flags & RAFTQ_SWEEP_VOTES) ? w : 0;
    counts->n_lost = (flags & RAFTQ_SWEEP_VOTES) ? l : 0;
  }
  if (want_list && segmented) {
    const uint64_t total = h->h_total[3] & 0xffffffffull;
    if (n_advanced) *n_advanced = total;
    h->adv_listed = total;
    h->adv_packed = true;
    h->adv_segmented = true;
  } else if (want_list) {
    const uint64_t total = *h->h_total;
    if (n_advanced) *n_advanced = total;
    const uint64_t take = std::min(total, take_cap);
    h->adv_listed = take;
    h->adv_packed = sizeof(Adv) == sizeof(Advance16);
    if (take && advances_out) std::memcpy(advances_out, h->adv.h, take * sizeof(Adv));
  }
  return verdict;
}

extern "C" {

int raftq_cycle(raftq_t* h, const raftq_delta_t* deltas, uint64_t n_deltas, const raftq_vote_delta_t* vote_deltas,
                uint64_t n_vote_deltas, unsigned flags, raftq_advance_t* advances_out, uint64_t cap,
                uint64_t* n_advanced, raftq_counts_t* counts) {
  return cycle_impl<DeltaRec, Advance>(h, "raftq_cycle", deltas, n_deltas, vote_deltas, n_vote_deltas, flags, advances_out, cap,
                                       n_advanced, counts);
}

int raftq_cycle_packed(raftq_t* h, const raftq_delta16_t* deltas, uint64_t n_deltas, const raftq_vote_delta_t* vote_deltas,
                       uint64_t n_vote_deltas, unsigned flags, raftq_advance16_t* advances_out, uint64_t cap,
                       uint64_t* n_advanced, raftq_counts_t* counts) {
  if (h && h->G > (1ull << 32))
    return fail(h, RAFTQ_EINVAL, "raftq_cycle_packed: the packed records carry 32-bit group ids (handle has more than 2^32 groups)");
  return cycle_impl<Delta16Rec, Advance16>(h, "raftq_cycle_packed", deltas, n_deltas, vote_deltas, n_vote_deltas, flags,
                                           advances_out, cap, n_advanced, counts);
}

int raftq_stage_packed(raftq_t* h, uint64_t n_deltas, uint64_t n_vote_deltas, raftq_delta16_t** deltas,
                       raftq_vote_delta_t** vote_deltas) {
  if (int rc = use_device_idle(h, "raftq_stage_packed")) return rc;
  const size_t off_votes = ((size_t)n_deltas * sizeof(raftq_delta16_t) + 255) / 256 * 256;
  if (int rc = ensure_ingest(h, off_votes + (size_t)n_vote_deltas * sizeof(raftq_vote_delta_t) + 256)) return rc;
  if (deltas) *deltas = (raftq_delta16_t*)h->ingest.h;
  if (vote_deltas) *vote_deltas = (raftq_vote_delta_t*)((uint8_t*)h->ingest.h + off_votes);
  return RAFTQ_OK;
}

int raftq_last_advances_packed(raftq_t* h, const raftq_advance16_t** list, uint64_t* n_listed) {
  if (!h) return fail(nullptr, RAFTQ_EINVAL, "null handle");
  if (!list || !n_listed) return fail(h, RAFTQ_EINVAL, "raftq_last_advances_packed: null argument");
  if (h->adv_listed && !h->adv_packed)
    return fail(h, RAFTQ_ESTATE, "raftq_last_advances_packed: the last list was produced in the 24-byte layout");
  if (h->adv_segmented)
    return fail(h, RAFTQ_ESTATE, "raftq_last_advances_packed: the last list lies in segments (raftq_last_advance_segments)");
  *list = (const raftq_advance16_t*)h->adv.h;
  *n_listed = h->adv_listed;
  return RAFTQ_OK;
}

int raftq_last_advance_segments(raftq_t* h, const raftq_advance16_t** recs, const uint32_t** counts, uint32_t* n_segments, uint64_t* stride) {
  if (!h) return fail(nullptr, RAFTQ_EINVAL, "null handle");
  if (!recs || !counts || !n_segments || !stride) return fail(h, RAFTQ_EINVAL, "raftq_last_advance_segments: null argument");
  if (h->adv_listed && !h->adv_packed)
    return fail(h, RAFTQ_ESTATE, "raftq_last_advance_segments: the last list was produced in the 24-byte layout");
  *recs = (const raftq_advance16_t*)h->adv.h;
  if (h->adv_segmented) {
    *counts = h->seg_h.h;
    *n_segments = h->seg_tiles;
    *stride = h->seg_stride;
  } else {
    h->seg_one = (uint32_t)h->adv_listed;
    *counts = &h->seg_one;
    *n_segments = 1;
    *stride = 0;
  }
  return RAFTQ_OK;
}

int raftq_timer_begin(raftq_t* h) {
  if (int rc = use_device(h)) return rc;
  HIPCHK(h, hipEventRecord(h->ev0, h->stream));
  return RAFTQ_OK;
}

int raftq_timer_end(raftq_t* h, float* elapsed_ms) {
  if (int rc = use_device(h)) return rc;
  if (!elapsed_ms) return fail(h, RAFTQ_EINVAL, "raftq_timer_end: null argument");
  HIPCHK(h, hipEventRecord(h->ev1, h->stream));
  HIPCHK(h, hipEventSynchronize(h->ev1));
  HIPCHK(h, hipEventElapsedTime(elapsed_ms, h->ev0, h->ev1));
  return RAFTQ_OK;
}

int raftq_host_alloc(void** p, uint64_t bytes) {
  if (!p || bytes == 0) return fail(nullptr, RAFTQ_EINVAL, "raftq_host_alloc: null pointer or zero size");
  *p = nullptr;
  int n = 0;
  if (hipGetDeviceCount(&n) != hipSuccess || n == 0) return fail(nullptr, RAFTQ_ENODEV, "raftq_host_alloc: no HIP device");
  const hipError_t e = hipHostMalloc(p, (size_t)bytes, hipHostMallocDefault);
  if (e != hipSuccess) {
    *p = nullptr;
    return fail(nullptr, e == hipErrorOutOfMemory ? RAFTQ_ENOMEM : RAFTQ_EHIP,
                std::string("raftq_host_alloc: ") + hipGetErrorString(e));
  }
  return RAFTQ_OK;
}

void raftq_host_free(void* p) {
  if (p) (void)hipHostFree(p);
}

}

namespace {
thread_local std::string g_set_err;
int sfail(raftq_set_t* s, int code, const std::string& msg) {
  g_set_err = msg;
  if (s) s->err = msg;
  return fail(nullptr, code, msg);
}
#define SETCHK(s, expr)                                                                                   \
  do {                                                                                                    \
// ... 277 lines not shown
    s->tick_since = 0;
  }
  const uint64_t n_blocks = s->gpad / 1024;
  int shape_now = 1;
  if (const char* e = std::getenv("RAFTQ_TICK_SHAPE"))
    shape_now = std::strcmp(e, "narrow") == 0 ? 0 : std::strcmp(e, "wide2") == 0 ? 2 : std::strcmp(e, "wide4") == 0 ? 4 : 1;
  auto wide_grid = [&](int r) { return dim3((unsigned)((n_blocks + (uint64_t)kWaves * r - 1) / ((uint64_t)kWaves * r)), (unsigned)K); };
  switch (shape_now) {
    case 0:
      hipLaunchKernelGGL(tick_set_kernel, dim3((unsigned)((n_blocks + kTickSetRounds - 1) / kTickSetRounds), (unsigned)K), dim3(kBlock), 0, s->stream,
                         (const TickArgs*)s->tick_tab, s->tick_since, n_blocks);
      break;
    case 2:
      hipLaunchKernelGGL((tick_set_wide_kernel<2>), wide_grid(2), dim3(kBlock), 0, s->stream, (const TickArgs*)s->tick_tab, s->tick_since, n_blocks);
      break;
    case 4:
      hipLaunchKernelGGL((tick_set_wide_kernel<4>), wide_grid(4), dim3(kBlock), 0, s->stream, (const TickArgs*)s->tick_tab, s->tick_since, n_blocks);
      break;
    default:
      hipLaunchKernelGGL((tick_set_wide_kernel<kTickWideBlocks>), wide_grid(kTickWideBlocks), dim3(kBlock), 0, s->stream, (const TickArgs*)s->tick_tab,
                         s->tick_since, n_blocks);
  }
  SETCHK(s, hipGetLastError());
  ++s->tick_since;
  for (raftq_t* h : s->members) {
    h->tl_valid = false;
    ++h->tick_no;
    h->ticked = true;
  }
  return RAFTQ_OK;
}

int raftq_set_wait(raftq_set_t* s, raftq_counts_t* per_member, raftq_counts_t* total) {
  if (int rc = set_ready(s, "raftq_set_wait")) return rc;
  const bool want = per_member || total;
  const size_t n = s->members.size();
  if (want) {
    if (!s->swept) return sfail(s, RAFTQ_ESTATE, "raftq_set_wait: no set sweep to report on");
    set_fill_table(s, -1, s->tab_host);
    SETCHK(s, hipMemcpyAsync(s->tab[2], s->tab_host.data(), n * sizeof(SweepArgs), hipMemcpyHostToDevice, s->stream));
    s->np_host.resize(n);
    for (size_t i = 0; i < n; ++i) s->np_host[i] = s->members[i]->n_partials;
    SETCHK(s, hipMemcpyAsync(s->np_d, s->np_host.data(), n * 8, hipMemcpyHostToDevice, s->stream));
    hipLaunchKernelGGL(set_counts_kernel, dim3((unsigned)n), dim3(kBlock), 0, s->stream, (const SweepArgs*)s->tab[2],
                       (const uint64_t*)s->np_d, s->counts_d);
    SETCHK(s, hipGetLastError());
    SETCHK(s, hipMemcpyAsync(s->counts_h, s->counts_d, n * 32, hipMemcpyDeviceToHost, s->stream));
  }
  SETCHK(s, hipStreamSynchronize(s->stream));
  if (want) {
    raftq_counts_t t{0, 0, 0};
    for (size_t i = 0; i < n; ++i) {
      const unsigned f = s->members[i]->last_flags;
      const bool commit = f & (RAFTQ_SWEEP_COMMIT | RAFTQ_SWEEP_GATED);
      const bool votes = f & RAFTQ_SWEEP_VOTES;
      raftq_counts_t c{commit ? s->counts_h[4 * i] : 0, votes ? s->counts_h[4 * i + 1] : 0, votes ? s->counts_h[4 * i + 2] : 0};
      if (per_member) per_member[i] = c;
      t.n_changed += c.n_changed;
      t.n_won += c.n_won;
      t.n_lost += c.n_lost;
    }
    if (total) *total = t;
  }
  return RAFTQ_OK;
}

int raftq_set_timer_begin(raftq_set_t* s) {
  if (int rc = set_ready(s, "raftq_set_timer_begin")) return rc;
  SETCHK(s, hipEventRecord(s->ev0, s->stream));
  return RAFTQ_OK;
}

int raftq_set_timer_end(raftq_set_t* s, float* elapsed_ms) {
  if (int rc = set_ready(s, "raftq_set_timer_end")) return rc;
  if (!elapsed_ms) return sfail(s, RAFTQ_EINVAL, "raftq_set_timer_end: null argument");
  SETCHK(s, hipEventRecord(s->ev1, s->stream));
  SETCHK(s, hipEventSynchronize(s->ev1));
  SETCHK(s, hipEventElapsedTime(elapsed_ms, s->ev0, s->ev1));
  return RAFTQ_OK;
}

int raftq_clone_state(raftq_t* dst, raftq_t* src) {
  if (int rc = use_device_idle(dst, "raftq_clone_state")) return rc;
  if (!src) return fail(dst, RAFTQ_EINVAL, "raftq_clone_state: null source");
  if (src == dst) return RAFTQ_OK;
  if (src->device != dst->device || src->N != dst->N || src->G != dst->G)
    return fail(dst, RAFTQ_EINVAL, "raftq_clone_state: source and destination must have the same device, groups and peers");
  if (src->step_collected != src->step_submitted)
    return fail(dst, RAFTQ_ESTATE, "raftq_clone_state: the source has Step batches in flight");
  if (src->voters && dst->in_set && !dst->in_set->allow_voters)
    return fail(dst, RAFTQ_ESTATE, "raftq_clone_state: the source has voter masks loaded and the destination is a member of a sweep "
                                   "set, whose dispatches count every slot (out of scope)");
  if (src->voters) {
    if (int rc = ensure_voters(dst)) return rc;
  } else if (int rc = drop_voters(dst)) {
    return rc;
  }
  HIPCHK(dst, hipStreamSynchronize(src->stream));
  const uint64_t ld = dst->ld;
  HIPCHK(dst, hipMemcpyAsync(dst->match, src->match, (size_t)dst->N * ld * 8, hipMemcpyDeviceToDevice, dst->stream));
  HIPCHK(dst, hipMemcpyAsync(dst->committed[dst->cur], src->committed[src->cur], ld * 8, hipMemcpyDeviceToDevice, dst->stream));
  HIPCHK(dst, hipMemcpyAsync(dst->first_idx, src->first_idx, ld * 8, hipMemcpyDeviceToDevice, dst->stream));
  HIPCHK(dst, hipMemcpyAsync(dst->votes, src->votes, (size_t)vote_word_bytes((int)dst->N) * ld, hipMemcpyDeviceToDevice,
                             dst->stream));
  HIPCHK(dst, hipMemcpyAsync(dst->self_max, src->self_max, sizeof(uint32_t), hipMemcpyDeviceToDevice, dst->stream));
  if (src->anchor && !dst->narrow_off && !dst->anchor) {
    if (raftq_buf::alloc_group({{(void**)&dst->anchor, ld * sizeof(uint64_t), raftq_buf::Kind::device, nullptr, false},
                                {(void**)&dst->moff, (size_t)dst->N * ld * sizeof(uint32_t), raftq_buf::Kind::device, nullptr, false}},
                               dst->stream) != hipSuccess)
      (void)hipGetLastError();
    else if (dst->in_set) dst->in_set->tab_stale = true;
  }
  if (src->anchor && dst->anchor && !dst->narrow_off) {
    HIPCHK(dst, hipMemcpyAsync(dst->anchor, src->anchor, ld * sizeof(uint64_t), hipMemcpyDeviceToDevice, dst->stream));
    HIPCHK(dst, hipMemcpyAsync(dst->moff, src->moff, (size_t)dst->N * ld * sizeof(uint32_t), hipMemcpyDeviceToDevice, dst->stream));
    HIPCHK(dst, hipMemcpyAsync(dst->narrow_word(), src->narrow_word(), sizeof(uint32_t), hipMemcpyDeviceToDevice, dst->stream));
  } else {
    HIPCHK(dst, hipMemsetAsync(dst->narrow_word(), 0, sizeof(uint32_t), dst->stream));
  }
  if (src->voters) HIPCHK(dst, hipMemcpyAsync(dst->voters, src->voters, ld * sizeof(uint16_t), hipMemcpyDeviceToDevice, dst->stream));
  if (src->cq && dst->cq) HIPCHK(dst, hipMemcpyAsync(dst->cq, src->cq, ld * sizeof(uint32_t), hipMemcpyDeviceToDevice, dst->stream));
  if (src->reads && dst->reads) HIPCHK(dst, hipMemcpyAsync(dst->reads, src->reads, ld * sizeof(raftqk::ReadRec), hipMemcpyDeviceToDevice, dst->stream));
  HIPCHK(dst, hipStreamSynchronize(dst->stream));
  dst->have_terms = src->have_terms;
  dense_changed(dst);
  return RAFTQ_OK;
}

}
```

raftsql_amd/csrc/raftq_internal.hpp:

```cpp
#pragma once
#include <hip/hip_runtime.h>

#include <string>
#include <vector>

#include "raftq.h"
#include "raftq_wire.h"
#include "raftq_kernels.hpp"
#include "raftq_buffers.hpp"

struct raftq {
  int device = 0;
  uint64_t G = 0, gpad = 0, ld = 0;
  uint32_t N = 0;
  hipStream_t stream = nullptr;
  bool own_stream = false;
  struct raftq_set* in_set = nullptr;
  uint64_t* match = nullptr;
  uint64_t* committed[2] = {nullptr, nullptr};
  int cur = 0;
  uint64_t* first_idx = nullptr;
  uint8_t* votes = nullptr;
  uint16_t* voters = nullptr;
  uint8_t* outcome = nullptr;
  uint64_t* changed_bits = nullptr;
  uint4* partials = nullptr;
  uint4* h_partials = nullptr;
  uint64_t n_partials = 0;
  uint64_t max_partials = 0;
  uint64_t* offsets = nullptr;
  uint64_t* h_total = nullptr;
  raftq_buf::Buffer<> stage{raftq_buf::Kind::mapped};
  raftq_buf::HostWritable ingest;
  raftq_buf::BarRule bar;
  std::vector<uint64_t> ld_mark, ld_start;
  struct LdNowait {
    raftq_buf::Buffer<> buf{raftq_buf::Kind::mapped};
    hipEvent_t ev = nullptr;
  };
  LdNowait ld_nowait[2];
  uint32_t ld_nowait_next = 0;
  std::vector<uint32_t> ld_round, ld_pos;
  uint32_t ld_epoch = 0;
  raftq_buf::Buffer<raftqk::Advance> adv{raftq_buf::Kind::mapped_coherent};
  uint64_t adv_listed = 0;
  bool adv_packed = false;
  bool adv_segmented = false;
  raftq_buf::Buffer<uint32_t> seg_h{raftq_buf::Kind::mapped_coherent};
  raftq_buf::Buffer<unsigned int> seg_d{raftq_buf::Kind::device};
  uint32_t seg_tiles = 0, seg_stride = 0, seg_one = 0;
  uint64_t flag_mask = ~0ull;
  uint32_t* self_max = nullptr;
  uint64_t* anchor = nullptr;
  uint32_t* moff = nullptr;
  bool narrow_off = false;
  uint32_t* narrow_word() const { return self_max + 1; }
  raftqk::NarrowMirror narrow_mirror() const { return raftqk::NarrowMirror{self_max + 1, anchor, moff}; }
  uint64_t compact_epoch = 0;
  uint64_t compact_epoch_armed = 0;
  uint32_t flag_misses[2] = {0, 0}, flag_rested[2] = {0, 0};
  uint64_t flag_fallbacks = 0;
  uint32_t* claim = nullptr;
  raftq_buf::Buffer<> delta_dev{raftq_buf::Kind::device};
  unsigned long long* delta_bad = nullptr;
  unsigned long long delta_epoch = 0;
  unsigned long long delta_check[2] = {0, 0};
  uint8_t* role = nullptr;
  uint32_t* elapsed = nullptr;
  uint8_t* action = nullptr;
  uint64_t* hup_bits = nullptr;
  uint64_t* beat_bits = nullptr;
  uint4* tick_partials = nullptr;
  raftq_buf::Buffer<uint32_t> tl{raftq_buf::Kind::mapped_coherent};
  uint64_t tl_hup_cap = 0, tl_beat_cap = 0, tl_beat_at = 0, tl_map_off = 0;
  uint64_t tl_n_hup = 0, tl_n_beat = 0;
  unsigned tl_flags = 0;
  bool tl_valid = false;
  uint64_t* tick_offsets2 = nullptr;
  uint32_t election_tick = 10, heartbeat_tick = 1;
  uint64_t tick_seed = 0x1000, tick_no = 0;
  bool ticked = false;
  uint32_t* cq = nullptr;
  uint64_t* chk_bits = nullptr;
  bool pre_vote = false;
  bool lead_transfer = false;
  uint8_t read_index = 0;
  void* reads = nullptr;
  uint64_t tick_chk_cap = 0;
  uint64_t tl_chk_cap = 0, tl_chk_off = 0, tl_n_chk = 0;
  bool tl_chk_valid = false;
  uint64_t* tick_offsets3 = nullptr;
  uint64_t* d_total = nullptr;
  bool have_terms = false;
  unsigned last_flags = 0;
  int last_gpl = 0;
  const uint64_t* last_old = nullptr;
  const uint64_t* last_new = nullptr;
  uint32_t self_peer = 0;
  bool self_set = false;
  bool node_mirror_fresh = false;
  uint64_t node_mirror_refreshes = 0;
  void* node_rec = nullptr;
  unsigned int* step_stall = nullptr;
  uint8_t step_compact = 0;
  bool step_msg_flags = false;
  bool step_voters = false;
  bool step_props = false;
  bool tick_voters = false;
  bool bcast_voters = false;
  bool resp_lead = false;
  bool resp_props = false;
  bool prop_forward = false;
  int step_walk_mode = 1;
  uint32_t step_stalls_in_a_row = 0, step_sorted_left = 0;
  uint64_t step_replays = 0;
  static constexpr int kStepSlots = 3;
  struct StepSlot {
    raftq_buf::Buffer<> in_h{raftq_buf::Kind::pinned};
    raftq_buf::HostWritable in_bar;
    raftq_buf::Buffer<> dev{raftq_buf::Kind::device};
    raftq_buf::Buffer<> out{raftq_buf::Kind::mapped};
    uint64_t n = 0;
    hipEvent_t ev_in = nullptr, ev_out = nullptr;
    bool busy = false;
    bool lists = false;
    bool replayed = false;
    bool copy_pending = false;
    const void* w_off_in_place = nullptr;
    const void* w_stream_in_place = nullptr;
    size_t w_stage_stream_off = 0;
    const void* msgs_in_place = nullptr;
    const void* outs_d = nullptr;
    uint64_t out_quads = 0;
    int end_bit = 0;
    uint32_t rec = 64;
    bool tail_zeroed = false;
    uint64_t tail_n = 0;
    uint32_t tail_rec = 0;
    const void* tail_dev = nullptr;
    uint64_t w_nbytes = 0;
// ... 159 lines not shown
```

raftsql_amd/csrc/raftq_kernels.hpp:

```cpp
#pragma once
#include <hip/hip_runtime.h>
#include <stdint.h>

#include <utility>

namespace raftqk {

typedef unsigned long long u64x2 __attribute__((ext_vector_type(2)));

constexpr int kBlock = 256;
constexpr int kWaves = kBlock / 64;
constexpr int kMaxPeers = 9;
constexpr int kTileMax = 2048;

struct __attribute__((aligned(64))) ReadRec {
  uint32_t seq;
  uint32_t acked[kMaxPeers];
  uint32_t pad[15 - kMaxPeers];
};
static_assert(sizeof(ReadRec) == 64, "one record per group, half a line");

struct SweepArgs {
  const uint64_t* match;
  const uint64_t* committed;
// ... 619 lines not shown
  }
}

struct DeltaRec {
  uint64_t group, match;
  uint32_t peer, pad;
};
struct Delta16Rec {
  uint64_t match;
  uint32_t group, peer;
};
struct VoteDeltaRec {
  uint64_t group;
  uint32_t peer;
  uint8_t vote, pad[3];
};

constexpr unsigned long long kNoEpoch = ~0ull;
__device__ __forceinline__ bool batch_is_bad(const unsigned long long* bad, unsigned long long epoch_match,
                                             unsigned long long epoch_votes) {
  return bad[0] == epoch_match || bad[1] == epoch_votes;
}

static __global__ __launch_bounds__(kBlock) void self_max_check_kernel(const uint64_t* __restrict__ match, uint64_t ld,
                                                                       uint64_t n_groups, uint32_t n_peers, uint32_t slot,
                                                                       uint32_t* word) {
  bool broken = false;
  for (uint64_t g = (uint64_t)blockIdx.x * kBlock + threadIdx.x; g < n_groups; g += (uint64_t)gridDim.x * kBlock) {
    const uint64_t own = match[(uint64_t)slot * ld + g];
    for (uint32_t p = 0; p < n_peers; ++p) broken |= match[(uint64_t)p * ld + g] > own;
  }
  if (__ballot(broken) != 0 && (threadIdx.x & 63) == 0) *word = 0u;
}

__device__ __forceinline__ bool breaks_self_max(uint32_t w, const uint64_t* match, uint64_t ld, uint64_t group, uint32_t peer,
                                                uint64_t value) {
  if ((w & kSelfMaxValid) == 0) return false;
  const uint32_t slot = w & 0xffu;
  return peer != slot && value > match[(uint64_t)slot * ld + group];
}
__device__ __forceinline__ void clear_self_max_if(bool broken, uint32_t* word) {
  const uint64_t b = __ballot(broken);
  if (b != 0 && (threadIdx.x & 63) == (uint32_t)(__ffsll((unsigned long long)b) - 1)) *word = 0u;
}

static __global__ __launch_bounds__(kBlock) void narrow_build_kernel(const uint64_t* __restrict__ match, uint64_t ld,
                                                                     uint64_t n_groups, uint32_t n_peers,
                                                                     uint64_t* __restrict__ anchor, uint32_t* __restrict__ moff,
                                                                     uint32_t* word) {
  bool broken = false;
  for (uint64_t g = (uint64_t)blockIdx.x * kBlock + threadIdx.x; g < n_groups; g += (uint64_t)gridDim.x * kBlock) {
    uint64_t lo = match[g], hi = lo;
    for (uint32_t p = 1; p < n_peers; ++p) {
      const uint64_t v = match[(uint64_t)p * ld + g];
      lo = v < lo ? v : lo;
      hi = v > hi ? v : hi;
    }
    anchor[g] = lo;
    if (hi - lo > 0xffffffffull) {
      broken = true;
    } else {
      for (uint32_t p = 0; p < n_peers; ++p) moff[(uint64_t)p * ld + g] = (uint32_t)(match[(uint64_t)p * ld + g] - lo);
    }
  }
  if (__ballot(broken) != 0 && (threadIdx.x & 63) == 0) *word = 0u;
}

struct NarrowMirror {
  uint32_t* word;
  const uint64_t* anchor;
  uint32_t* moff;
};
__device__ __forceinline__ bool narrow_follow(uint32_t w, const NarrowMirror& m, uint64_t ld, uint64_t group, uint32_t peer,
                                              uint64_t value) {
  if (w != kNarrowValid) return false;
  const uint64_t base = m.anchor[group];
  if (value < base) return false;
  if (value - base > 0xffffffffull) return true;
  atomicMax(m.moff + (uint64_t)peer * ld + group, (uint32_t)(value - base));
  return false;
}
__device__ __forceinline__ void clear_narrow_if(bool broken, uint32_t* word) { clear_self_max_if(broken, word); }

template <typename Rec>
static __global__ __launch_bounds__(kBlock) void deltas_in_kernel(const Rec* __restrict__ src, Rec* __restrict__ dst,
                                                                  uint64_t n, uint64_t n_groups, uint32_t n_peers,
                                                                  unsigned long long* bad_epoch, uint64_t* bad_host,
                                                                  unsigned long long epoch) {
  const uint64_t i = (uint64_t)blockIdx.x * kBlock + threadIdx.x;
  bool bad = false;
  if (i < n) {
    const Rec r = src[i];
    dst[i] = r;
    bad = r.group >= n_groups || r.peer >= n_peers;
  }
  if (__ballot(bad) != 0 && (threadIdx.x & 63) == 0) {
    atomicMax(bad_epoch, epoch);
    *bad_host = epoch;
  }
}

template <typename Rec>
static __global__ __launch_bounds__(kBlock) void deltas_in_apply_kernel(const Rec* __restrict__ src, uint64_t n, uint64_t* match,
                                                                        uint64_t ld, uint64_t n_groups, uint32_t n_peers,
                                                                        unsigned long long* bad_epoch, uint64_t* bad_host,
                                                                        unsigned long long epoch, uint32_t* self_max,
                                                                        NarrowMirror mirror) {
  const uint64_t i = (uint64_t)blockIdx.x * kBlock + threadIdx.x;
  const uint32_t w = *self_max;
  const uint32_t nw = *mirror.word;
  bool bad = false, broken = false, wide = false;
  if (i < n) {
    const Rec r = src[i];
    bad = r.group >= n_groups || r.peer >= n_peers;
    if (!bad) {
      broken = breaks_self_max(w, match, ld, r.group, r.peer, r.match);
      wide = narrow_follow(nw, mirror, ld, r.group, r.peer, r.match);
      atomicMax(reinterpret_cast<unsigned long long*>(match + (uint64_t)r.peer * ld + r.group), (unsigned long long)r.match);
    }
  }
  clear_self_max_if(broken, self_max);
  clear_narrow_if(wide, mirror.word);
  if (__ballot(bad) != 0 && (threadIdx.x & 63) == 0) {
    atomicMax(bad_epoch, epoch);
    *bad_host = epoch;
  }
}

template <typename Rec>
static __global__ __launch_bounds__(kBlock) void apply_deltas_kernel(uint64_t* match, uint64_t ld,
                                                              const Rec* __restrict__ d, uint64_t n,
                                                              const unsigned long long* bad,
                                                              unsigned long long epoch_match, unsigned long long epoch_votes,
                                                              uint32_t* self_max, NarrowMirror mirror) {
  if (batch_is_bad(bad, epoch_match, epoch_votes)) return;
  const uint64_t i = (uint64_t)blockIdx.x * kBlock + threadIdx.x;
  const uint32_t w = *self_max;
  const uint32_t nw = *mirror.word;
  bool broken = false, wide = false;
  if (i < n) {
    const Rec r = d[i];
    broken = breaks_self_max(w, match, ld, r.group, r.peer, r.match);
    wide = narrow_follow(nw, mirror, ld, r.group, r.peer, r.match);
    atomicMax(reinterpret_cast<unsigned long long*>(match + (uint64_t)r.peer * ld + r.group),
              (unsigned long long)r.match);
  }
  clear_self_max_if(broken, self_max);
  clear_narrow_if(wide, mirror.word);
}

struct TermDeltaRec {
  uint64_t group, cur_term, first_idx_cur_term;
};
static __global__ __launch_bounds__(kBlock) void apply_term_deltas_kernel(uint64_t* first_idx,
                                                                   const TermDeltaRec* __restrict__ d, uint64_t n) {
  const uint64_t i = (uint64_t)blockIdx.x * kBlock + threadIdx.x;
  if (i >= n) return;
  const TermDeltaRec r = d[i];
  first_idx[r.group] = r.cur_term == 0 ? 0ull : r.first_idx_cur_term;
}

static __global__ __launch_bounds__(kBlock) void vote_deltas_in_kernel(const VoteDeltaRec* __restrict__ src,
                                                                       VoteDeltaRec* __restrict__ dst, uint64_t n,
                                                                       uint64_t n_groups, uint32_t n_peers,
                                                                       unsigned long long* bad_epoch, uint64_t* bad_host,
                                                                       unsigned long long epoch) {
  const uint64_t i = (uint64_t)blockIdx.x * kBlock + threadIdx.x;
  bool bad = false;
  if (i < n) {
    const VoteDeltaRec r = src[i];
    dst[i] = r;
    bad = r.group >= n_groups || r.peer >= n_peers || (unsigned)(r.vote - 1) > 1u;
  }
  if (__ballot(bad) != 0 && (threadIdx.x & 63) == 0) {
    atomicMax(bad_epoch, epoch);
    *bad_host = epoch;
  }
}

__device__ __forceinline__ bool vote_rec_ok(const VoteDeltaRec& r, uint64_t n_groups, uint32_t n_peers) {
  return r.group < n_groups && r.peer < n_peers && (unsigned)(r.vote - 1) <= 1u;
}

static __global__ __launch_bounds__(kBlock) void vote_claim_kernel(uint32_t* claim, uint64_t ld,
                                                            const VoteDeltaRec* __restrict__ d, uint64_t n,
                                                            const unsigned long long* bad, unsigned long long epoch_match,
                                                            unsigned long long epoch_votes, uint64_t n_groups,
                                                            uint32_t n_peers, int each) {
  if (!each && batch_is_bad(bad, epoch_match, epoch_votes)) return;
  const uint64_t i = (uint64_t)blockIdx.x * kBlock + threadIdx.x;
  if (i >= n) return;
  const VoteDeltaRec r = d[i];
  if (each && !vote_rec_ok(r, n_groups, n_peers)) return;
  atomicMin(claim + (uint64_t)r.peer * ld + r.group, (uint32_t)i);
}

static __global__ __launch_bounds__(kBlock) void vote_apply_kernel(uint8_t* votes, int wide, uint32_t* claim, uint64_t ld,
                                                            const VoteDeltaRec* __restrict__ d, uint64_t n,
                                                            const unsigned long long* bad, unsigned long long epoch_match,
                                                            unsigned long long epoch_votes, uint64_t n_groups,
                                                            uint32_t n_peers, int each) {
  if (!each && batch_is_bad(bad, epoch_match, epoch_votes)) return;
  const uint64_t i = (uint64_t)blockIdx.x * kBlock + threadIdx.x;
  if (i >= n) return;
  const VoteDeltaRec r = d[i];
  if (each && !vote_rec_ok(r, n_groups, n_peers)) return;
  const uint64_t slot = (uint64_t)r.peer * ld + r.group;
  if (claim[slot] != (uint32_t)i) return;
  unsigned int* word = reinterpret_cast<unsigned int*>(votes) + (wide ? r.group : r.group >> 1);
  const unsigned sh = (wide ? 0u : (unsigned)(r.group & 1ull) * 16u) + 2u * r.peer;
  const unsigned nv = (unsigned)r.vote << sh;
  unsigned old = *word;
  while (true) {
    const unsigned cur = (old >> sh) & 3u;
    if (cur == 1u || cur == 2u) break;
    const unsigned seen = atomicCAS(word, old, (old & ~(3u << sh)) | nv);
    if (seen == old) break;
    old = seen;
  }
  claim[slot] = 0xffffffffu;
}

struct Advance {
  uint64_t group, old_commit, new_commit;
};
struct Advance16 {
  uint64_t new_commit;
  uint32_t group, advanced_by;
};
// ... 103 lines not shown
      const uint64_t g = g0 + 2 * lane, s = pos + rank;
      if (s < cap) out[s] = make_advance((Adv*)nullptr, g, old_commit[g], new_commit[g]);
    }
    if (o) {
      const uint64_t g = g0 + 2 * lane + 1, s = pos + rank + (e ? 1 : 0);
      if (s < cap) out[s] = make_advance((Adv*)nullptr, g, old_commit[g], new_commit[g]);
    }
    pos += __popcll(b0) + __popcll(b1);
  }
}

static __global__ void raise_flag_kernel(uint64_t* flag, uint64_t epoch) {
  if (threadIdx.x == 0 && blockIdx.x == 0) __hip_atomic_store(flag, epoch, __ATOMIC_RELAXED, __HIP_MEMORY_SCOPE_SYSTEM);
}

template <int N, int GPL, bool GATED, int POLICY>
static __global__ __launch_bounds__(kBlock) void sweep_segments_kernel(SweepArgs a, Advance16* list, unsigned int* counts_host, unsigned int* counts_dev) {
  constexpr bool STNT = (POLICY & kStNT) != 0;
  constexpr int kTile = kBlock * GPL;
  constexpr int kRounds = GPL / 2;
  __shared__ uint32_t wave_cnt[kWaves];
  const uint32_t tid = threadIdx.x, lane = tid & 63, wave = tid >> 6, tile = blockIdx.x;
  TileRegs<N, GPL, true, GATED, false> r;
  r.skip = tile_body<N, true>(a);
  const bool narrow = N >= 3 && r.skip == kSkipNarrow;
  if (narrow) {
    if constexpr (N >= 3) tile_load<N, GPL, true, GATED, false, POLICY, kBlock, kBodyNarrow>(r, a, tile);
  } else if (r.skip != 0) {
    tile_load<N, GPL, true, GATED, false, POLICY, kBlock, kBodySkip>(r, a, tile);
  } else {
    tile_load<N, GPL, true, GATED, false, POLICY>(r, a, tile);
  }
  const uint64_t tile0 = (uint64_t)tile * kTile;
  u64x2 nw[kRounds];
  uint64_t even[kRounds], odd[kRounds];
  uint32_t n_changed = 0;
#pragma unroll
  for (int j = 0; j < kRounds; ++j) {
    const uint64_t g = tile0 + (uint64_t)wave * (64 * GPL) + (uint64_t)j * 128 + 2 * lane;
    uint64_t mci0 = 0, mci1 = 0;
    if (narrow) {
      if constexpr (N >= 3) tile_mci<N, kBodyNarrow, false>(r, j, mci0, mci1);
    } else if (r.skip != 0) {
      tile_mci<N, kBodySkip, false>(r, j, mci0, mci1);
    } else {
      tile_mci<N, kBodyAll, false>(r, j, mci0, mci1);
    }
    u64x2 o;
    o.x = maybe_commit<GATED>(mci0, r.c[j].x, GATED ? r.f[j].x : 0);
    o.y = maybe_commit<GATED>(mci1, r.c[j].y, GATED ? r.f[j].y : 0);
    even[j] = __ballot(o.x != r.c[j].x);
    odd[j] = __ballot(o.y != r.c[j].y);
    n_changed += __popcll(even[j]) + __popcll(odd[j]);
    nw[j] = o;
    if (a.changed_bits != nullptr && lane == 0) {
      u64x2 w;
      w.x = even[j];
      w.y = odd[j];
      stg<false>(reinterpret_cast<u64x2*>(a.changed_bits + (g >> 6)), w);
    }
    stg<STNT>(reinterpret_cast<u64x2*>(a.committed_out + g), o);
  }
  if (lane == 0) {
    uint4 t;
    t.x = n_changed;
    t.y = t.z = t.w = 0;
    stg_u4(a.partials + ((uint64_t)tile * kWaves + wave), t);
    wave_cnt[wave] = n_changed;
  }
  __syncthreads();
  uint64_t pos = tile0;
  for (uint32_t k = 0; k < wave; ++k) pos += wave_cnt[k];
  if (tid == 0) {
    uint32_t tile_cnt = 0;
#pragma unroll
    for (int k = 0; k < kWaves; ++k) tile_cnt += wave_cnt[k];
    counts_host[tile] = tile_cnt;
    counts_dev[tile] = tile_cnt;
  }
  const uint64_t below = lane == 0 ? 0ull : (~0ull >> (64 - lane));
#pragma unroll
  for (int j = 0; j < kRounds; ++j) {
    const uint64_t g0 = tile0 + (uint64_t)wave * (64 * GPL) + (uint64_t)j * 128;
    const bool e = (even[j] >> lane) & 1, o = (odd[j] >> lane) & 1;
    const uint64_t rank = __popcll(even[j] & below) + __popcll(odd[j] & below);
    if (e) list[pos + rank] = make_advance((Advance16*)nullptr, g0 + 2 * lane, r.c[j].x, nw[j].x);
    if (o) list[pos + rank + (e ? 1 : 0)] = make_advance((Advance16*)nullptr, g0 + 2 * lane + 1, r.c[j].y, nw[j].y);
    pos += __popcll(even[j]) + __popcll(odd[j]);
  }
}

static __global__ __launch_bounds__(kBlock) void raise_flag_segments_kernel(uint64_t* flag, uint32_t epoch, const unsigned int* counts_dev, uint32_t n_tiles) {
  __shared__ uint32_t red[kWaves];
  uint32_t acc = 0;
  for (uint32_t i = threadIdx.x; i < n_tiles; i += kBlock) acc += counts_dev[i];
#pragma unroll
  for (int o = 32; o > 0; o >>= 1) acc += __shfl_xor(acc, o, 64);
  if ((threadIdx.x & 63) == 0) red[threadIdx.x >> 6] = acc;
  __syncthreads();
  if (threadIdx.x == 0) {
    uint32_t total = 0;
#pragma unroll
    for (int k = 0; k < kWaves; ++k) total += red[k];
    __hip_atomic_store(flag, ((uint64_t)epoch << 32) | total, __ATOMIC_RELAXED, __HIP_MEMORY_SCOPE_SYSTEM);
  }
}

struct VoterSweepArgs {
  SweepArgs s;
  const uint16_t* voters;
};

__device__ __forceinline__ uint64_t sel_u64(bool c, uint64_t a, uint64_t b) { return c ? a : b; }

template <int N, int... I>
__device__ __forceinline__ uint64_t pick_sorted(const uint64_t (&v)[N], uint32_t idx, std::integer_sequence<int, I...>) {
  uint64_t r = v[0];
  ((r = sel_u64(idx == (uint32_t)(I + 1), v[I + 1], r)), ...);
  return r;
}
template <int N, int... I>
__device__ __forceinline__ void zero_non_voters(uint64_t (&v)[N], uint32_t mask, std::integer_sequence<int, I...>) {
  ((v[I] = sel_u64(((mask >> I) & 1u) != 0, v[I], 0ull)), ...);
}

template <int N>
__device__ __forceinline__ uint64_t select_quorum_voters(uint64_t (&v)[N], uint32_t mask) {
  zero_non_voters<N>(v, mask, std::make_integer_sequence<int, N>{});
  if constexpr (N >= 2) (void)select_quorum_network<N>(v);
  return pick_sorted<N>(v, (uint32_t)__popc(mask) >> 1, std::make_integer_sequence<int, N - 1>{});
}

__device__ __forceinline__ uint32_t spread_even(uint32_t m) {
  m = (m | (m << 8)) & 0x00ff00ffu;
  m = (m | (m << 4)) & 0x0f0f0f0fu;
  m = (m | (m << 2)) & 0x33333333u;
  return (m | (m << 1)) & 0x55555555u;
}

__device__ __forceinline__ uint32_t poll_word_voters(uint32_t w, uint32_t mask) {
  const uint32_t low = spread_even(mask);
  const uint32_t q = ((uint32_t)__popc(mask) >> 1) + 1u;
  const uint32_t granted = __popc(w & ~(w >> 1) & low);
  const uint32_t rejected = __popc((w >> 1) & ~w & low);
  const uint32_t won = granted >= q ? 1u : 0u;
  const uint32_t lost = (won == 0u && rejected >= q) ? 2u : 0u;
  return won | lost;
}

template <int N, int GPL, bool COMMIT, bool GATED, bool VOTES, int POLICY>
static __global__ __launch_bounds__(kBlock) void sweep_voters_kernel(VoterSweepArgs va) {
#define RAFTQ_VT_PROLOGUE      \
  const SweepArgs& a = va.s; \
  const uint32_t tid = threadIdx.x, tile = blockIdx.x;
#define RAFTQ_VT_VMASK(at) ldg<NT>(reinterpret_cast<const u32x4p*>(va.voters + at))
#define RAFTQ_VT_CMASK(j, at) ldg<NT>(reinterpret_cast<const uint32_t*>(va.voters + at))
#include "raftq_sweep_voters_tile.inc"
#undef RAFTQ_VT_PROLOGUE
#undef RAFTQ_VT_VMASK
#undef RAFTQ_VT_CMASK
}

template <int GPL, bool COMMIT>
struct TileMasks {
  u32x4p v;
  uint32_t c[COMMIT ? GPL / 2 : 1];
// ... 537 lines not shown
```

raftsql_amd/engine.py:

```python
from __future__ import annotations

import ctypes as C
from dataclasses import dataclass
from typing import Optional

import numpy as np

from . import _lib
from ._lib import (SWEEP_CACHED, SWEEP_CHANGED, SWEEP_COMMIT, SWEEP_GATED, SWEEP_LDS, SWEEP_NO_ADOPT,
                   SWEEP_STREAM, SWEEP_VOTES, Advance, Counts, Delta, RaftqError, VoteDelta)

__all__ = ["QuorumEngine", "SweepSet", "sweep_many_async", "SweepCounts", "device_count", "RaftqError", "pinned_empty", "pinned_copy", "SWEEP_COMMIT", "SWEEP_GATED",
           "SWEEP_VOTES", "SWEEP_NO_ADOPT", "SWEEP_LDS", "SWEEP_CHANGED", "SWEEP_STREAM", "SWEEP_CACHED"]


@dataclass
class SweepCounts:
    n_changed: int
    n_won: int
    n_lost: int


def device_count() -> int:
    lib = _lib.load()
# ... 268 lines not shown
        nv = 0 if vote_deltas is None else len(vote_deltas)
        n = C.c_uint64(0)
        self._chk(self._lib.raftq_cycle(
            self._h, _ptr(deltas) if nd else None, nd, _ptr(vote_deltas) if nv else None, nv, flags,
            None, int(cap), C.byref(n), None))
        return int(n.value)

    def cycle(self, flags: int, deltas: Optional[np.ndarray] = None, vote_deltas: Optional[np.ndarray] = None,
              cap: Optional[int] = None, out: Optional[np.ndarray] = None, want_counts: bool = True):
        nd = 0 if deltas is None else len(deltas)
        nv = 0 if vote_deltas is None else len(vote_deltas)
        if nd:
            assert deltas.dtype == self._DELTA_DT and deltas.flags.c_contiguous
        if nv:
            assert vote_deltas.dtype == self._VDELTA_DT and vote_deltas.flags.c_contiguous
        cap = (self.n_groups if cap is None else int(cap))
        if out is None:
            out = np.empty(cap, dtype=self._ADV_DT)
        n = C.c_uint64(0)
        c = Counts()
        self._chk(self._lib.raftq_cycle(
            self._h, _ptr(deltas) if nd else None, nd, _ptr(vote_deltas) if nv else None, nv, flags,
            _ptr(out) if cap else None, cap, C.byref(n), C.byref(c) if want_counts else None))
        total = int(n.value)
        cnt = SweepCounts(int(c.n_changed), int(c.n_won), int(c.n_lost)) if want_counts else None
        return out[: min(total, cap)], total, cnt

    def step_async(self, flags: int) -> None:
        self._chk(self._lib.raftq_step_async(self._h, flags))

    def wait(self, want_counts: bool = False) -> Optional[SweepCounts]:
        if not want_counts:
            self._chk(self._lib.raftq_wait(self._h, None))
            return None
        c = Counts()
        self._chk(self._lib.raftq_wait(self._h, C.byref(c)))
        return SweepCounts(int(c.n_changed), int(c.n_won), int(c.n_lost))

    def sweep(self, flags: int) -> SweepCounts:
        self.step_async(flags)
        return self.wait(want_counts=True)

    def commit_advance(self, gated: bool = False):
        out = np.empty(self.n_groups, dtype=np.uint64)
        n = C.c_uint64(0)
        self._chk(self._lib.raftq_commit_advance(self._h, int(gated), _ptr(out), C.byref(n)))
        return out, int(n.value)

    def vote_tally(self):
        out = np.empty(self.n_groups, dtype=np.uint8)
        c = Counts()
        self._chk(self._lib.raftq_vote_tally(self._h, _ptr(out), C.byref(c)))
        return out, SweepCounts(int(c.n_changed), int(c.n_won), int(c.n_lost))

    def read_committed(self) -> np.ndarray:
        out = np.empty(self.n_groups, dtype=np.uint64)
        self._chk(self._lib.raftq_read_committed(self._h, _ptr(out)))
        return out

    def read_outcome(self) -> np.ndarray:
        out = np.empty(self.n_groups, dtype=np.uint8)
        self._chk(self._lib.raftq_read_outcome(self._h, _ptr(out)))
        return out

    def read_match(self) -> np.ndarray:
        out = np.empty((self.n_peers, self.n_groups), dtype=np.uint64)
        self._chk(self._lib.raftq_read_match(self._h, _ptr(out)))
        return out

    def self_max(self) -> int:
        s = C.c_int32(-1)
        self._chk(self._lib.raftq_self_max(self._h, C.byref(s)))
        return int(s.value)

    def narrow(self) -> bool:
        v = C.c_int32(0)
        self._chk(self._lib.raftq_narrow(self._h, C.byref(v)))
        return bool(v.value)

    def narrow_rebuild(self) -> bool:
        self._chk(self._lib.raftq_narrow_rebuild(self._h))
        return self.narrow()

    def read_votes(self) -> np.ndarray:
        out = np.empty((self.n_peers, self.n_groups), dtype=np.uint8)
        self._chk(self._lib.raftq_read_votes(self._h, _ptr(out)))
        return out

    def collect_changed(self, cap: Optional[int] = None):
        cap = self.n_groups if cap is None else int(cap)
        arr = (Advance * cap)()
        n = C.c_uint64(0)
        self._chk(self._lib.raftq_collect_changed(self._h, C.addressof(arr) if cap else None, cap, C.byref(n)))
        a = np.frombuffer(arr, dtype=np.dtype([("group", "<u8"), ("old_commit", "<u8"), ("new_commit", "<u8")]))
        return a[: min(int(n.value), cap)].copy(), int(n.value)

    def set_timers(self, election_tick: int = 10, heartbeat_tick: int = 1, seed: int = 0x1000) -> None:
        self._chk(self._lib.raftq_set_timers(self._h, election_tick, heartbeat_tick, seed))

    def load_roles(self, role: np.ndarray, elapsed: Optional[np.ndarray] = None) -> None:
        r = np.ascontiguousarray(role, dtype=np.uint8)
        if r.shape != (self.n_groups,):
            raise ValueError("role must be [G]")
        e = None if elapsed is None else np.ascontiguousarray(elapsed, dtype=np.uint32)
        self._chk(self._lib.raftq_load_roles(self._h, _ptr(r), _ptr(e) if e is not None else None))

    def tick(self, want_counts: bool = True):
        if not want_counts:
            self._chk(self._lib.raftq_tick(self._h, None))
            return None
        c = _lib.TickCounts()
        self._chk(self._lib.raftq_tick(self._h, C.byref(c)))
        return int(c.n_hup), int(c.n_beat)

    def read_tick(self):
        a = np.empty(self.n_groups, dtype=np.uint8)
        e = np.empty(self.n_groups, dtype=np.uint32)
        r = np.empty(self.n_groups, dtype=np.uint8)
        self._chk(self._lib.raftq_read_tick(self._h, _ptr(a), _ptr(e), _ptr(r)))
        return a, e, r

    def collect_hups(self, cap: Optional[int] = None):
        cap = self.n_groups if cap is None else int(cap)
        out = np.empty(cap, dtype=np.uint64)
        n = C.c_uint64(0)
        self._chk(self._lib.raftq_collect_hups(self._h, _ptr(out) if cap else None, cap, C.byref(n)))
        return out[: min(cap, int(n.value))], int(n.value)

    def collect_beats(self, cap: Optional[int] = None):
        cap = self.n_groups if cap is None else int(cap)
        out = np.empty(cap, dtype=np.uint64)
        n = C.c_uint64(0)
        self._chk(self._lib.raftq_collect_beats(self._h, _ptr(out) if cap else None, cap, C.byref(n)))
        return out[: min(cap, int(n.value))], int(n.value)

    def set_check_quorum(self, on=True) -> None:
        self._chk(self._lib.raftq_set_check_quorum(self._h, int(on)))

    def set_pre_vote(self, on=True) -> None:
        self._chk(self._lib.raftq_set_pre_vote(self._h, int(on)))

    def set_lead_transfer(self, on=True) -> None:
        self._chk(self._lib.raftq_set_lead_transfer(self._h, int(on)))

    def load_transfer(self, transferee: np.ndarray) -> None:
        t = np.ascontiguousarray(transferee, dtype=np.uint8)
        if t.shape != (self.n_groups,):
            raise ValueError("transferee must be [G]")
        self._chk(self._lib.raftq_load_transfer(self._h, _ptr(t)))

    def read_transfer(self) -> np.ndarray:
        t = np.empty(self.n_groups, dtype=np.uint8)
        self._chk(self._lib.raftq_read_transfer(self._h, _ptr(t)))
        return t

    def set_read_index(self, mode=_lib.READ_SAFE) -> None:
        self._chk(self._lib.raftq_set_read_index(self._h, int(mode)))

    def load_reads(self, seq: Optional[np.ndarray] = None, acked: Optional[np.ndarray] = None) -> None:
        s = None if seq is None else np.ascontiguousarray(seq, dtype=np.uint32)
        a = None if acked is None else np.ascontiguousarray(acked, dtype=np.uint32)
        if s is not None and s.shape != (self.n_groups,):
            raise ValueError("seq must be [G]")
        if a is not None and a.shape != (self.n_peers, self.n_groups):
            raise ValueError("acked must be [N][G]")
        self._chk(self._lib.raftq_load_reads(self._h, None if s is None else _ptr(s), None if a is None else _ptr(a)))
# ... 164 lines not shown
```

Before: 130.5 billion.

## Mark touched groups during delta ingest and sweep only marked pairs

Adds a per-group dirty bitmap that the delta-apply kernels set with atomicOr, and a marked segmented sweep kernel that loads match rows only for groups marked this turn. Committed values are loaded only for groups that are marked or changed last turn. The fast path is used only when the previous cycle was of the same kind and no intervening API call invalidated state, which is tracked through a turn_clean word. This saves memory bandwidth on sparse updates, at the cost of atomics during ingest, a bitmap memset, and fragile state tracking across API calls.

```diff
diff --git a/go/raftq/engine_more.go b/go/raftq/engine_more.go
--- a/go/raftq/engine_more.go
+++ b/go/raftq/engine_more.go
@@ -28,6 +28,14 @@
 }
 
 func (e *Engine) NarrowRebuild() error { return e.err(C.raftq_narrow_rebuild(e.h)) }
+
+func (e *Engine) TurnMarked() (int, error) {
+	var state C.int32_t
+	if err := e.err(C.raftq_turn_marked(e.h, &state)); err != nil {
+		return 0, err
+	}
+	return int(state), nil
+}
 
 func (e *Engine) SetStream(stream unsafe.Pointer) error { return e.err(C.raftq_set_stream(e.h, stream)) }
 func (e *Engine) Stream() unsafe.Pointer                { return C.raftq_get_stream(e.h) }
diff --git a/include/raftq.h b/include/raftq.h
--- a/include/raftq.h
+++ b/include/raftq.h
@@ -122,6 +122,7 @@
 int raftq_self_max(raftq_t* h, int32_t* slot_out);
 int raftq_narrow(raftq_t* h, int32_t* valid_out);
 int raftq_narrow_rebuild(raftq_t* h);
+int raftq_turn_marked(raftq_t* h, int32_t* state_out);
 int raftq_read_votes(raftq_t* h, uint8_t* votes_out );
 int raftq_collect_changed(raftq_t* h, raftq_advance_t* out, uint64_t cap, uint64_t* n);
 
diff --git a/raftsql_amd/_lib.py b/raftsql_amd/_lib.py
--- a/raftsql_amd/_lib.py
+++ b/raftsql_amd/_lib.py
@@ -81,6 +81,7 @@
     ("raftq_self_max", C.c_int, [_H, C.POINTER(C.c_int32)]),
     ("raftq_narrow", C.c_int, [_H, C.POINTER(C.c_int32)]),
     ("raftq_narrow_rebuild", C.c_int, [_H]),
+    ("raftq_turn_marked", C.c_int, [_H, C.POINTER(C.c_int32)]),
     ("raftq_read_votes", C.c_int, [_H, C.c_void_p]),
     ("raftq_collect_changed", C.c_int, [_H, C.c_void_p, C.c_uint64, C.POINTER(C.c_uint64)]),
     ("raftq_set_timers", C.c_int, [_H, C.c_uint32, C.c_uint32, C.c_uint64]),
diff --git a/raftsql_amd/csrc/raftq_capi.hip b/raftsql_amd/csrc/raftq_capi.hip
--- a/raftsql_amd/csrc/raftq_capi.hip
+++ b/raftsql_amd/csrc/raftq_capi.hip
@@ -162,6 +162,19 @@
   });
 }
 
+hipError_t launch_segments_marked(uint32_t N, const SweepArgs& a, uint64_t* marks, uint32_t n_tiles, bool gated, int nt, Advance16* list,
+                                  unsigned int* counts_host, unsigned int* counts_dev, hipStream_t s) {
+  const dim3 grid(n_tiles), block(kBlock);
+  return with_peers(N, [&](auto n) {
+    return with_policy(nt, [&](auto pol) {
+      constexpr int NP = decltype(n)::value, POLICY = decltype(pol)::value;
+      if (gated) hipLaunchKernelGGL((sweep_segments_marked_kernel<NP, kGPL, true, POLICY>), grid, block, 0, s, a, marks, list, counts_host, counts_dev);
+      else hipLaunchKernelGGL((sweep_segments_marked_kernel<NP, kGPL, false, POLICY>), grid, block, 0, s, a, marks, list, counts_host, counts_dev);
+      return hipGetLastError();
+    });
+  });
+}
+
 constexpr int voters_gpl(int n_peers) { return n_peers <= 6 ? 4 : 2; }
 
 hipError_t launch_voters(uint32_t N, const VoterSweepArgs& a, uint64_t gpad, unsigned flags, int nt, hipStream_t s) {
@@ -260,8 +273,21 @@
 }
 int raftq_detail::use_device(raftq_t* h) {
   if (!h) return fail(nullptr, RAFTQ_EINVAL, "null handle");
+  h->turn_clean = 0;
   HIPCHK(h, hipSetDevice(h->device));
   return RAFTQ_OK;
+}
+namespace {
+struct KeepTurnClean {
+  raftq_t* h;
+  int word;
+  explicit KeepTurnClean(raftq_t* h_) : h(h_), word(h_ ? h_->turn_clean : 0) {}
+  ~KeepTurnClean() {
+    if (h) h->turn_clean = word;
+  }
+  KeepTurnClean(const KeepTurnClean&) = delete;
+  KeepTurnClean& operator=(const KeepTurnClean&) = delete;
+};
 }
 int raftq_detail::use_device_idle(raftq_t* h, const char* who) {
   if (int rc = use_device(h)) return rc;
@@ -370,6 +396,8 @@
     {
       const char* nr = std::getenv("RAFTQ_NARROW");
       h->narrow_off = nr && std::strcmp(nr, "0") == 0;
+      const char* tm = std::getenv("RAFTQ_TURN_MARKED");
+      h->turn_marked_off = tm && std::strcmp(tm, "0") == 0;
     }
     e = hipMemsetD32Async((hipDeviceptr_t)h->self_max, (int)(kSelfMaxValid | 0u), 1, h->stream);
     if (e != hipSuccess) { rc = fail(h, RAFTQ_EHIP, std::string("hipMemsetD32Async: ") + hipGetErrorString(e)); break; }
@@ -417,7 +445,7 @@
   raftq_detail::free_node_state(h);
   raftq_detail::free_wire_state(h);
   raftq_buf::free_device(h->match, h->committed[0], h->committed[1], h->first_idx, h->votes, h->voters, h->outcome, h->changed_bits,
-                         h->partials, h->offsets, h->self_max, h->anchor, h->moff, h->claim, h->delta_bad, h->role, h->elapsed, h->action, h->hup_bits,
+                         h->partials, h->offsets, h->self_max, h->anchor, h->moff, h->marks, h->claim, h->delta_bad, h->role, h->elapsed, h->action, h->hup_bits,
                          h->beat_bits, h->tick_partials, h->tick_offsets2, h->tick_offsets3, h->cq, h->chk_bits, h->reads);
   raftq_buf::free_host(h->h_partials, h->h_total);
   if (h->ev0) (void)hipEventDestroy(h->ev0);
@@ -517,7 +545,7 @@
 
 template <typename Rec, typename AbiRec>
 static int enqueue_ingest(raftq_t* h, const AbiRec* d, uint64_t n, const raftq_vote_delta_t* vd, uint64_t nv, size_t off_votes,
-                          bool trusted = false) {
+                          bool trusted = false, uint64_t* marks = nullptr ) {
   static_assert(sizeof(Rec) == sizeof(AbiRec), "ABI struct mismatch");
   static_assert(sizeof(VoteDeltaRec) == sizeof(raftq_vote_delta_t), "ABI struct mismatch");
   if (nv > 0xfffffffeull) return fail(h, RAFTQ_EINVAL, "vote delta batch too large");
@@ -553,7 +581,7 @@
   if (n) dense_changed(h);
   if (n && trusted)
     hipLaunchKernelGGL((deltas_in_apply_kernel<Rec>), gm, dim3(kBlock), 0, h->stream, (const Rec*)h->ingest.d, n, h->match, h->ld,
-                       h->G, h->N, h->delta_bad, h->d_total + 1, em, h->self_max, h->narrow_mirror());
+                       h->G, h->N, h->delta_bad, h->d_total + 1, em, h->self_max, h->narrow_mirror(), marks);
   else if (n)
     hipLaunchKernelGGL((deltas_in_kernel<Rec>), gm, dim3(kBlock), 0, h->stream, (const Rec*)h->ingest.d, dev_m, n, h->G, h->N,
                        h->delta_bad, h->d_total + 1, em);
@@ -563,7 +591,7 @@
                        h->d_total + 2, ev);
   if (n && !trusted)
     hipLaunchKernelGGL((apply_deltas_kernel<Rec>), gm, dim3(kBlock), 0, h->stream, h->match, h->ld, (const Rec*)dev_m, n, bad, em,
-                       ev, h->self_max, h->narrow_mirror());
+                       ev, h->self_max, h->narrow_mirror(), marks);
   if (nv) {
     const unsigned long long em_gate = trusted ? kNoEpoch : em;
     hipLaunchKernelGGL(vote_claim_kernel, gv, dim3(kBlock), 0, h->stream, h->claim, h->ld, (const VoteDeltaRec*)dev_v, nv, bad,
@@ -778,6 +806,7 @@
 static void sweep_done(raftq_t* h, unsigned flags, int gpl) {
   const bool commit = flags & (RAFTQ_SWEEP_COMMIT | RAFTQ_SWEEP_GATED);
   h->n_partials = h->gpad / ((uint64_t)kBlock * gpl) * kWaves;
+  h->turn_clean = 0;
   h->last_flags = flags;
   h->last_gpl = gpl;
   if (commit) {
@@ -872,6 +901,7 @@
 }
 
 int raftq_read_committed(raftq_t* h, uint64_t* out) {
+  KeepTurnClean keep(h);
   if (int rc = use_device_idle(h, "raftq_read_committed")) return rc;
   if (!out) return fail(h, RAFTQ_EINVAL, "raftq_read_committed: null argument");
   const uint64_t* src = (h->last_flags & RAFTQ_SWEEP_NO_ADOPT) && h->last_new ? h->last_new : h->committed[h->cur];
@@ -896,6 +926,7 @@
 }
 
 int raftq_self_max(raftq_t* h, int32_t* slot) {
+  KeepTurnClean keep(h);
   if (int rc = use_device_idle(h, "raftq_self_max")) return rc;
   if (!slot) return fail(h, RAFTQ_EINVAL, "raftq_self_max: null argument");
   uint32_t w = 0;
@@ -906,12 +937,20 @@
 }
 
 int raftq_narrow(raftq_t* h, int32_t* valid) {
+  KeepTurnClean keep(h);
   if (int rc = use_device_idle(h, "raftq_narrow")) return rc;
   if (!valid) return fail(h, RAFTQ_EINVAL, "raftq_narrow: null argument");
   uint32_t w = 0;
   HIPCHK(h, hipMemcpyAsync(&w, h->narrow_word(), sizeof w, hipMemcpyDeviceToHost, h->stream));
   HIPCHK(h, hipStreamSynchronize(h->stream));
   *valid = w == kNarrowValid ? 1 : 0;
+  return RAFTQ_OK;
+}
+
+int raftq_turn_marked(raftq_t* h, int32_t* state_out) {
+  if (!h) return fail(nullptr, RAFTQ_EINVAL, "null handle");
+  if (!state_out) return fail(h, RAFTQ_EINVAL, "raftq_turn_marked: null argument");
+  *state_out = h->turn_clean;
   return RAFTQ_OK;
 }
 
@@ -1691,7 +1730,7 @@
   if (h->voters) return false;
   return (flags & (RAFTQ_SWEEP_COMMIT | RAFTQ_SWEEP_GATED)) && !(flags & ~allowed) && h->gpad <= kSegmentsMaxGroups;
 }
-static int enqueue_sweep_segments(raftq_t* h, unsigned flags) {
+static int enqueue_sweep_segments(raftq_t* h, unsigned flags, bool marked) {
   const uint32_t n_tiles = (uint32_t)(h->gpad / kTile);
   if (int rc = ensure_adv(h, (h->gpad * sizeof(Advance16) + sizeof(Advance) - 1) / sizeof(Advance))) return rc;
   HIPCHK(h, h->seg_h.grow((size_t)n_tiles * 4, (size_t)n_tiles * 4, &h->stream));
@@ -1699,8 +1738,12 @@
   const SweepArgs a = sweep_args(h, h->cur, true);
   uint64_t epoch = ++h->compact_epoch;
   if ((uint32_t)epoch == 0) epoch = ++h->compact_epoch;
-  HIPCHK(h, launch_segments(h->N, a, n_tiles, (flags & RAFTQ_SWEEP_GATED) != 0, sweep_policy(flags, sweep_footprint(h)), (Advance16*)h->adv.d, h->seg_h.d,
-                            h->seg_d.d, h->stream));
+  if (marked)
+    HIPCHK(h, launch_segments_marked(h->N, a, h->marks, n_tiles, (flags & RAFTQ_SWEEP_GATED) != 0, sweep_policy(flags, sweep_footprint(h)),
+                                     (Advance16*)h->adv.d, h->seg_h.d, h->seg_d.d, h->stream));
+  else
+    HIPCHK(h, launch_segments(h->N, a, n_tiles, (flags & RAFTQ_SWEEP_GATED) != 0, sweep_policy(flags, sweep_footprint(h)), (Advance16*)h->adv.d, h->seg_h.d,
+                              h->seg_d.d, h->stream));
   sweep_done(h, flags, kGPL);
   hipLaunchKernelGGL(raise_flag_segments_kernel, dim3(1), dim3(kBlock), 0, h->stream, h->d_total + 3, (uint32_t)epoch, h->seg_d.d, n_tiles);
   HIPCHK(h, hipGetLastError());
@@ -1714,6 +1757,7 @@
 extern "C" {
 
 int raftq_collect_changed(raftq_t* h, raftq_advance_t* out, uint64_t cap, uint64_t* n) {
+  KeepTurnClean keep(h);
   if (int rc = use_device_idle(h, "raftq_collect_changed")) return rc;
   if (!n) return fail(h, RAFTQ_EINVAL, "raftq_collect_changed: null count");
   if (!(h->last_flags & RAFTQ_SWEEP_CHANGED) || !h->last_old)
@@ -1740,6 +1784,7 @@
 
 int raftq_stage(raftq_t* h, uint64_t n_deltas, uint64_t n_vote_deltas, raftq_delta_t** deltas,
                 raftq_vote_delta_t** vote_deltas) {
+  KeepTurnClean keep(h);
   if (int rc = use_device_idle(h, "raftq_stage")) return rc;
   const size_t off_votes = vote_stage_offset(n_deltas);
   if (int rc = ensure_ingest(h, off_votes + (size_t)n_vote_deltas * sizeof(raftq_vote_delta_t) + 256)) return rc;
@@ -1796,10 +1841,23 @@
   return e;
 }
 
+static size_t marks_bytes(const raftq_t* h) { return (size_t)(h->ld / 64 + 2) * sizeof(uint64_t); }
+static bool turn_marks_ready(raftq_t* h) {
+  if (h->turn_marked_off || h->marks_failed) return false;
+  if (h->marks) return true;
+  if (raftq_buf::alloc_zeroed((void**)&h->marks, marks_bytes(h), h->stream) != hipSuccess) {
+    (void)hipGetLastError();
+    h->marks_failed = true;
+    return false;
+  }
+  return true;
+}
+
 template <typename Rec, typename Adv, typename AbiRec, typename AbiAdv>
 static int cycle_impl(raftq_t* h, const char* who, const AbiRec* deltas, uint64_t n_deltas, const raftq_vote_delta_t* vote_deltas,
                       uint64_t n_vote_deltas, unsigned flags, AbiAdv* advances_out, uint64_t cap, uint64_t* n_advanced,
                       raftq_counts_t* counts) {
+  const int clean_in = h ? h->turn_clean : 0;
   if (int rc = use_device_idle(h, who)) return rc;
   if ((n_deltas && !deltas) || (n_vote_deltas && !vote_deltas))
     return fail(h, RAFTQ_EINVAL, std::string(who) + ": null array with non-zero length");
@@ -1828,16 +1886,22 @@
   const auto t0 = clk::now();
   const bool trusted = flags & RAFTQ_CYCLE_TRUSTED;
   flags &= ~RAFTQ_CYCLE_TRUSTED;
+  const bool flag_wake = want_list && !counts;
+  const bool segmented = want_segments && flag_wake && !advances_out && sizeof(Adv) == sizeof(Advance16) && segments_ok(h, flags);
+  const int kind = !segmented || (flags & RAFTQ_SWEEP_NO_ADOPT) ? 0 : (flags & RAFTQ_SWEEP_GATED) ? 2 : 1;
+  const bool marked = kind != 0 && clean_in == kind && turn_marks_ready(h);
+  if (marked) {
+    if (h->marks_dirty) HIPCHK(h, hipMemsetAsync(h->marks, 0, marks_bytes(h), h->stream));
+    h->marks_dirty = true;
+  }
   if (n_deltas || n_vote_deltas)
-    if (int rc = enqueue_ingest<Rec>(h, deltas, n_deltas, vote_deltas, n_vote_deltas, off_votes, trusted)) return rc;
+    if (int rc = enqueue_ingest<Rec>(h, deltas, n_deltas, vote_deltas, n_vote_deltas, off_votes, trusted, marked ? h->marks : nullptr)) return rc;
   const auto t1 = clk::now();
   const int cur_before = h->cur;
-  const bool flag_wake = want_list && !counts;
-  const bool segmented = want_segments && flag_wake && !advances_out && sizeof(Adv) == sizeof(Advance16) && segments_ok(h, flags);
   h->flag_mask = ~0ull;
   h->adv_segmented = false;
   if (segmented) {
-    if (int rc = enqueue_sweep_segments(h, flags | RAFTQ_SWEEP_CHANGED)) return rc;
+    if (int rc = enqueue_sweep_segments(h, flags | RAFTQ_SWEEP_CHANGED, marked)) return rc;
   } else if (int rc = raftq_step_async(h, flags)) {
     return rc;
   }
@@ -1849,6 +1913,7 @@
                              h->stream));
   const auto t3 = clk::now();
   HIPCHK(h, wait_turn(h, flag_wake ? h->compact_epoch_armed : 0));
+  if (marked) h->marks_dirty = false;
   if (flag_wake && h->compact_epoch_armed) {
     static const bool check = [] { const char* e = std::getenv("RAFTQ_CYCLE_CHECK"); return e && e[0] == '1'; }();
     if (check) {
@@ -1916,6 +1981,7 @@
     h->adv_packed = sizeof(Adv) == sizeof(Advance16);
     if (take && advances_out) std::memcpy(advances_out, h->adv.h, take * sizeof(Adv));
   }
+  if (verdict == RAFTQ_OK && !h->turn_marked_off) h->turn_clean = kind;
   return verdict;
 }
 
@@ -1939,6 +2005,7 @@
 
 int raftq_stage_packed(raftq_t* h, uint64_t n_deltas, uint64_t n_vote_deltas, raftq_delta16_t** deltas,
                        raftq_vote_delta_t** vote_deltas) {
+  KeepTurnClean keep(h);
   if (int rc = use_device_idle(h, "raftq_stage_packed")) return rc;
   const size_t off_votes = ((size_t)n_deltas * sizeof(raftq_delta16_t) + 255) / 256 * 256;
   if (int rc = ensure_ingest(h, off_votes + (size_t)n_vote_deltas * sizeof(raftq_vote_delta_t) + 256)) return rc;
@@ -2382,6 +2449,7 @@
 
 int raftq_clone_state(raftq_t* dst, raftq_t* src) {
   if (int rc = use_device_idle(dst, "raftq_clone_state")) return rc;
+  dst->turn_clean = 0;
   if (!src) return fail(dst, RAFTQ_EINVAL, "raftq_clone_state: null source");
   if (src == dst) return RAFTQ_OK;
   if (src->device != dst->device || src->N != dst->N || src->G != dst->G)
diff --git a/raftsql_amd/csrc/raftq_internal.hpp b/raftsql_amd/csrc/raftq_internal.hpp
--- a/raftsql_amd/csrc/raftq_internal.hpp
+++ b/raftsql_amd/csrc/raftq_internal.hpp
@@ -56,6 +56,11 @@
   bool narrow_off = false;
   uint32_t* narrow_word() const { return self_max + 1; }
   raftqk::NarrowMirror narrow_mirror() const { return raftqk::NarrowMirror{self_max + 1, anchor, moff}; }
+  int turn_clean = 0;
+  uint64_t* marks = nullptr;
+  bool marks_failed = false;
+  bool marks_dirty = false;
+  bool turn_marked_off = false;
   uint64_t compact_epoch = 0;
   uint64_t compact_epoch_armed = 0;
   uint32_t flag_misses[2] = {0, 0}, flag_rested[2] = {0, 0};
diff --git a/raftsql_amd/csrc/raftq_kernels.hpp b/raftsql_amd/csrc/raftq_kernels.hpp
--- a/raftsql_amd/csrc/raftq_kernels.hpp
+++ b/raftsql_amd/csrc/raftq_kernels.hpp
@@ -725,6 +725,17 @@
 }
 __device__ __forceinline__ void clear_narrow_if(bool broken, uint32_t* word) { clear_self_max_if(broken, word); }
 
+__device__ __forceinline__ void mark_groups(uint64_t* marks, bool applied, uint64_t group) {
+  if (marks == nullptr) return;
+  const unsigned long long mine = applied ? (unsigned long long)group : ~0ull;
+  const unsigned long long left = __shfl_up(mine, 1, 64);
+  if (applied && ((threadIdx.x & 63) == 0 || left != mine)) {
+    const uint64_t word = 2 * (group >> 7) + (group & 1);
+    const uint32_t bit = (uint32_t)(group & 127) >> 1;
+    atomicOr(reinterpret_cast<unsigned int*>(marks) + 2 * word + (bit >> 5), 1u << (bit & 31));
+  }
+}
+
 template <typename Rec>
 static __global__ __launch_bounds__(kBlock) void deltas_in_kernel(const Rec* __restrict__ src, Rec* __restrict__ dst,
                                                                   uint64_t n, uint64_t n_groups, uint32_t n_peers,
@@ -748,11 +759,12 @@
                                                                         uint64_t ld, uint64_t n_groups, uint32_t n_peers,
                                                                         unsigned long long* bad_epoch, uint64_t* bad_host,
                                                                         unsigned long long epoch, uint32_t* self_max,
-                                                                        NarrowMirror mirror) {
+                                                                        NarrowMirror mirror, uint64_t* marks) {
   const uint64_t i = (uint64_t)blockIdx.x * kBlock + threadIdx.x;
   const uint32_t w = *self_max;
   const uint32_t nw = *mirror.word;
   bool bad = false, broken = false, wide = false;
+  uint64_t applied_group = 0;
   if (i < n) {
     const Rec r = src[i];
     bad = r.group >= n_groups || r.peer >= n_peers;
@@ -760,8 +772,10 @@
       broken = breaks_self_max(w, match, ld, r.group, r.peer, r.match);
       wide = narrow_follow(nw, mirror, ld, r.group, r.peer, r.match);
       atomicMax(reinterpret_cast<unsigned long long*>(match + (uint64_t)r.peer * ld + r.group), (unsigned long long)r.match);
-    }
-  }
+      applied_group = r.group;
+    }
+  }
+  mark_groups(marks, i < n && !bad, applied_group);
   clear_self_max_if(broken, self_max);
   clear_narrow_if(wide, mirror.word);
   if (__ballot(bad) != 0 && (threadIdx.x & 63) == 0) {
@@ -775,19 +789,22 @@
                                                               const Rec* __restrict__ d, uint64_t n,
                                                               const unsigned long long* bad,
                                                               unsigned long long epoch_match, unsigned long long epoch_votes,
-                                                              uint32_t* self_max, NarrowMirror mirror) {
+                                                              uint32_t* self_max, NarrowMirror mirror, uint64_t* marks) {
   if (batch_is_bad(bad, epoch_match, epoch_votes)) return;
   const uint64_t i = (uint64_t)blockIdx.x * kBlock + threadIdx.x;
   const uint32_t w = *self_max;
   const uint32_t nw = *mirror.word;
   bool broken = false, wide = false;
+  uint64_t applied_group = 0;
   if (i < n) {
     const Rec r = d[i];
     broken = breaks_self_max(w, match, ld, r.group, r.peer, r.match);
     wide = narrow_follow(nw, mirror, ld, r.group, r.peer, r.match);
     atomicMax(reinterpret_cast<unsigned long long*>(match + (uint64_t)r.peer * ld + r.group),
               (unsigned long long)r.match);
-  }
+    applied_group = r.group;
+  }
+  mark_groups(marks, i < n, applied_group);
   clear_self_max_if(broken, self_max);
   clear_narrow_if(wide, mirror.word);
 }
@@ -1057,6 +1074,137 @@
 #pragma unroll
   for (int j = 0; j < kRounds; ++j) {
     const uint64_t g0 = tile0 + (uint64_t)wave * (64 * GPL) + (uint64_t)j * 128;
+    const bool e = (even[j] >> lane) & 1, o = (odd[j] >> lane) & 1;
+    const uint64_t rank = __popcll(even[j] & below) + __popcll(odd[j] & below);
+    if (e) list[pos + rank] = make_advance((Advance16*)nullptr, g0 + 2 * lane, r.c[j].x, nw[j].x);
+    if (o) list[pos + rank + (e ? 1 : 0)] = make_advance((Advance16*)nullptr, g0 + 2 * lane + 1, r.c[j].y, nw[j].y);
+    pos += __popcll(even[j]) + __popcll(odd[j]);
+  }
+}
+
+template <int N, int GPL, bool GATED, int POLICY, int BODY>
+__device__ __forceinline__ void pair_load_match(TileRegs<N, GPL, true, GATED, false>& r, const SweepArgs& a, const int j, const uint64_t g) {
+  constexpr bool NT = (POLICY & kLdNT) != 0;
+  if constexpr (BODY == kBodyNarrow) {
+#pragma unroll
+    for (int p = 0; p < N; ++p) {
+      const uint64_t w = ldg<NT>(reinterpret_cast<const uint64_t*>(a.moff + (uint64_t)p * a.ld + g));
+      if (p & 1) r.m[j][p >> 1].y = w;
+      else r.m[j][p >> 1].x = w;
+    }
+    r.m[j][N - 1] = ldg<NT>(reinterpret_cast<const u64x2*>(a.anchor + g));
+  } else {
+    constexpr bool SKIP = BODY == kBodySkip;
+    constexpr int kRows = SKIP && N >= 2 ? N - 1 : N;
+#pragma unroll
+    for (int p = 0; p < kRows; ++p) {
+      const uint32_t slot = SKIP ? (uint32_t)p + ((uint32_t)p + 1 >= r.skip ? 1u : 0u) : (uint32_t)p;
+      r.m[j][p] = ldg<NT>(reinterpret_cast<const u64x2*>(a.match + (uint64_t)slot * a.ld + g));
+    }
+  }
+}
+
+template <int N, int GPL, bool GATED, int POLICY>
+static __global__ __launch_bounds__(kBlock) void sweep_segments_marked_kernel(SweepArgs a, uint64_t* marks, Advance16* list, unsigned int* counts_host,
+                                                                              unsigned int* counts_dev) {
+  constexpr bool NT = (POLICY & kLdNT) != 0;
+  constexpr bool STNT = (POLICY & kStNT) != 0;
+  constexpr int kTile = kBlock * GPL;
+  constexpr int kRounds = GPL / 2;
+  __shared__ uint32_t wave_cnt[kWaves];
+  const uint32_t tid = threadIdx.x, lane = tid & 63, wave = tid >> 6, tile = blockIdx.x;
+  const uint64_t tile0 = (uint64_t)tile * kTile;
+  const uint64_t wave0 = tile0 + (uint64_t)wave * (64 * GPL);
+  u64x2 mk[kRounds], pv[kRounds];
+#pragma unroll
+  for (int j = 0; j < kRounds; ++j) {
+    const uint64_t w = (wave0 + (uint64_t)j * 128) >> 6;
+    mk[j] = ldg<false>(reinterpret_cast<const u64x2*>(marks + w));
+    pv[j] = ldg<false>(reinterpret_cast<const u64x2*>(a.changed_bits + w));
+  }
+  TileRegs<N, GPL, true, GATED, false> r;
+  r.skip = tile_body<N, true>(a);
+  const bool narrow = N >= 3 && r.skip == kSkipNarrow;
+  uint64_t mk_any[kRounds], c_any[kRounds];
+#pragma unroll
+  for (int j = 0; j < kRounds; ++j) {
+    mk_any[j] = mk[j].x | mk[j].y;
+    c_any[j] = mk_any[j] | pv[j].x | pv[j].y;
+  }
+#pragma unroll
+  for (int j = 0; j < kRounds; ++j) {
+    const uint64_t g = wave0 + (uint64_t)j * 128 + 2 * lane;
+    r.c[j].x = r.c[j].y = 0;
+    if ((c_any[j] >> lane) & 1) {
+      r.c[j] = ldg<NT>(reinterpret_cast<const u64x2*>(a.committed + g));
+      if constexpr (GATED) r.f[j] = ldg<NT>(reinterpret_cast<const u64x2*>(a.first_idx + g));
+    }
+    if ((mk_any[j] >> lane) & 1) {
+      if (narrow) {
+        if constexpr (N >= 3) pair_load_match<N, GPL, GATED, POLICY, kBodyNarrow>(r, a, j, g);
+      } else if (r.skip != 0) {
+        pair_load_match<N, GPL, GATED, POLICY, kBodySkip>(r, a, j, g);
+      } else {
+        pair_load_match<N, GPL, GATED, POLICY, kBodyAll>(r, a, j, g);
+      }
+    }
+  }
+  u64x2 nw[kRounds];
+  uint64_t even[kRounds], odd[kRounds];
+  uint32_t n_changed = 0;
+#pragma unroll
+  for (int j = 0; j < kRounds; ++j) {
+    const uint64_t g = wave0 + (uint64_t)j * 128 + 2 * lane;
+    u64x2 o = r.c[j];
+    if ((mk_any[j] >> lane) & 1) {
+      uint64_t mci0 = 0, mci1 = 0;
+      if (narrow) {
+        if constexpr (N >= 3) tile_mci<N, kBodyNarrow, false>(r, j, mci0, mci1);
+      } else if (r.skip != 0) {
+        tile_mci<N, kBodySkip, false>(r, j, mci0, mci1);
+      } else {
+        tile_mci<N, kBodyAll, false>(r, j, mci0, mci1);
+      }
+      o.x = maybe_commit<GATED>(mci0, r.c[j].x, GATED ? r.f[j].x : 0);
+      o.y = maybe_commit<GATED>(mci1, r.c[j].y, GATED ? r.f[j].y : 0);
+    }
+    even[j] = __ballot(o.x != r.c[j].x);
+    odd[j] = __ballot(o.y != r.c[j].y);
+    n_changed += __popcll(even[j]) + __popcll(odd[j]);
+    nw[j] = o;
+    if (lane == 0) {
+      u64x2 w;
+      w.x = even[j];
+      w.y = odd[j];
+      stg<false>(reinterpret_cast<u64x2*>(a.changed_bits + (g >> 6)), w);
+      if (mk_any[j] != 0) {
+        w.x = w.y = 0;
+        stg<false>(reinterpret_cast<u64x2*>(marks + (g >> 6)), w);
+      }
+    }
+    if ((c_any[j] >> lane) & 1) stg<STNT>(reinterpret_cast<u64x2*>(a.committed_out + g), o);
+  }
+  if (lane == 0) {
+    uint4 t;
+    t.x = n_changed;
+    t.y = t.z = t.w = 0;
+    stg_u4(a.partials + ((uint64_t)tile * kWaves + wave), t);
+    wave_cnt[wave] = n_changed;
+  }
+  __syncthreads();
+  uint64_t pos = tile0;
+  for (uint32_t k = 0; k < wave; ++k) pos += wave_cnt[k];
+  if (tid == 0) {
+    uint32_t tile_cnt = 0;
+#pragma unroll
+    for (int k = 0; k < kWaves; ++k) tile_cnt += wave_cnt[k];
+    counts_host[tile] = tile_cnt;
+    counts_dev[tile] = tile_cnt;
+  }
+  const uint64_t below = lane == 0 ? 0ull : (~0ull >> (64 - lane));
+#pragma unroll
+  for (int j = 0; j < kRounds; ++j) {
+    const uint64_t g0 = wave0 + (uint64_t)j * 128;
     const bool e = (even[j] >> lane) & 1, o = (odd[j] >> lane) & 1;
     const uint64_t rank = __popcll(even[j] & below) + __popcll(odd[j] & below);
     if (e) list[pos + rank] = make_advance((Advance16*)nullptr, g0 + 2 * lane, r.c[j].x, nw[j].x);
diff --git a/raftsql_amd/engine.py b/raftsql_amd/engine.py
--- a/raftsql_amd/engine.py
+++ b/raftsql_amd/engine.py
@@ -374,6 +374,11 @@
         self._chk(self._lib.raftq_narrow_rebuild(self._h))
         return self.narrow()
 
+    def turn_marked(self) -> int:
+        v = C.c_int32(0)
+        self._chk(self._lib.raftq_turn_marked(self._h, C.byref(v)))
+        return int(v.value)
+
     def read_votes(self) -> np.ndarray:
         out = np.empty((self.n_peers, self.n_groups), dtype=np.uint8)
         self._chk(self._lib.raftq_read_votes(self._h, _ptr(out)))
```

Result: no change. 130.7 billion (median of 3 runs) (+0.2%).
